# 34j/vr180-convert

Measured on NVIDIA B200. Metric: SBS equirect output Mpix/s, higher is better.
Workload: dtype f64 coordinates / u8 fixed-point (INTER_BITS=5) sampling

## Files before the change

### vr180-convert_b200/csrc/chain_fast.cuh

```cuda
#pragma once
#include "chain.cuh"

namespace vr180 {

static __device__ const double2 kAsinTab[92] = {
    {0x1.0000000000000p+0, 0x0.0p+0},
    {0x1.fffbfffbfff80p-1, 0x1.0000aaabdde0cp-7},
    {0x1.ffefffbffdfffp-1, 0x1.0002aabdde94cp-6},
    {0x1.ffdbfebbe9360p-1, 0x1.80090091d9024p-6},
    {0x1.ffbffbff7fec0p-1, 0x1.000aabde0b9c8p-5},
    {0x1.ff9bf63a1740bp-1, 0x1.4014d8ffaf8afp-5},
    {0x1.ff6febba4bfeap-1, 0x1.8024091fdb0a9p-5},
    {0x1.ff3bda6d9c950p-1, 0x1.c0393e65c2c93p-5},
    {0x1.feffbfdfebf1fp-1, 0x1.002abde953619p-4},
    {0x1.febb993aecf99p-1, 0x1.203ce2b380cd3p-4},
    {0x1.fe6f634576477p-1, 0x1.405390240e6fdp-4},
    {0x1.fe1b1a62bddadp-1, 0x1.606f49730ccc5p-4},
    {0x1.fdbeba917c3f5p-1, 0x1.809092913e52ep-4},
    {0x1.fd5a3f6af6b74p-1, 0x1.a0b7f03ba78acp-4},
    {0x1.fceda421efdb5p-1, 0x1.c0e5e80f7172dp-4},
    {0x1.fc78e3817e16ep-1, 0x1.e11b009e269b5p-4},
    {0x1.fbfbf7ebc755fp-1, 0x1.00abe0c129e1ep-3},
    {0x1.fb76db58a1299p-1, 0x1.10ce59ba4a8c4p-3},
    {0x1.fae987541497fp-1, 0x1.20f530308cc20p-3},
    {0x1.fa53f4fcc4b79p-1, 0x1.3120a9bed2f46p-3},
    {0x1.f9b61d0237250p-1, 0x1.41510cb011423p-3},
    {0x1.f90ff7a2fd4d2p-1, 0x1.5186a00ade974p-3},
    {0x1.f8617caabd6f6p-1, 0x1.61c1ab9d55d30p-3},
    {0x1.f7aaa3701a270p-1, 0x1.720278094cd3cp-3},
    {0x1.f6eb62d27730dp-1, 0x1.82494ed0e78fcp-3},
    {0x1.f623b1379a09bp-1, 0x1.92967a638db38p-3},
    {0x1.f553848924e81p-1, 0x1.a2ea462b4998ep-3},
    {0x1.f47ad231ea746p-1, 0x1.b344fe9a97c4dp-3},
    {0x1.f3998f1b1886cp-1, 0x1.c3a6f13aae84bp-3},
    {0x1.f2afafa9380f9p-1, 0x1.d4106cba45b08p-3},
    {0x1.f1bd27b9002c4p-1, 0x1.e481c0fce7134p-3},
    {0x1.f0c1ea9bfa45fp-1, 0x1.f4fb3f2ad079bp-3},
    {0x1.efbdeb14f4edap-1, 0x1.02be9ce0b87cdp-2},
    {0x1.eeb11b5442ff1p-1, 0x1.0b04025245cccp-2},
    {0x1.ed9b6cf3c4663p-1, 0x1.134dfa9805147p-2},
    {0x1.ec7cd0f2b5ae0p-1, 0x1.1b9cb12545e62p-2},
    {0x1.eb5537b1434dap-1, 0x1.23f0523c5dc2bp-2},
    {0x1.ea2490ebdd6b8p-1, 0x1.2c490af8bde81p-2},
    {0x1.e8eacbb648910p-1, 0x1.34a709597aab1p-2},
    {0x1.e7a7d6766784bp-1, 0x1.3d0a7c4c4bd9cp-2},
    {0x1.e65b9edeba38ep-1, 0x1.457393b90e2aap-2},
    {0x1.e50611e88d6b5p-1, 0x1.4de2808dce513p-2},
    {0x1.e3a71bcdd63dep-1, 0x1.565774cb66f02p-2},
    {0x1.e23ea802b4b1ap-1, 0x1.5ed2a392bb50fp-2},
    {0x1.e0cca12e97895p-1, 0x1.675441329986ep-2},
    {0x1.df50f124fba75p-1, 0x1.6fdc83364f719p-2},
    {0x1.ddcb80ddc085bp-1, 0x1.786ba074fef93p-2},
    {0x1.dc3c386d0ae09p-1, 0x1.8101d121bed2dp-2},
    {0x1.daa2fefaae1d8p-1, 0x1.899f4edc962d3p-2},
    {0x1.d8ffbab9145d4p-1, 0x1.924454c462cc4p-2},
    {0x1.d75250db9c792p-1, 0x1.9af11f89ba61cp-2},
    {0x1.d59aa58c6471cp-1, 0x1.a3a5ed82d9537p-2},
    {0x1.d3d89be176072p-1, 0x1.ac62fec0b2a92p-2},
    {0x1.d20c15d14a4e5p-1, 0x1.b5289525368abp-2},
    {0x1.d034f42698214p-1, 0x1.bdf6f47ae6904p-2},
    {0x1.ce5316736032ep-1, 0x1.c6ce628dd132cp-2},
    {0x1.cc665b0328622p-1, 0x1.cfaf27460fe9fp-2},
    {0x1.ca6e9ecc569b9p-1, 0x1.d8998cc3e6049p-2},
    {0x1.c86bbd609a260p-1, 0x1.e18ddf7da106bp-2},
    {0x1.c65d90dc509f4p-1, 0x1.ea8c6e5f5e67fp-2},
    {0x1.c443f1d4d22afp-1, 0x1.f3958aecddef4p-2},
    {0x1.c21eb7458e5ccp-1, 0x1.fca989658baafp-2},
    {0x1.bfedb67be13b3p-1, 0x1.02e46075785a1p-1},
    {0x1.bdb0c30185485p-1, 0x1.0779c5d4df4b8p-1},
    {0x1.bb67ae8584caap-1, 0x1.0c152382d7366p-1},
    {0x1.b91248c38986bp-1, 0x1.10b6a9e43942fp-1},
    {0x1.b6b05f6966b9bp-1, 0x1.155e8b2a00052p-1},
    {0x1.b441bdfab5580p-1, 0x1.1a0cfb6c3e9ebp-1},
    {0x1.b1c62db2564fep-1, 0x1.1ec230c714a96p-1},
    {0x1.af3d7561a9c43p-1, 0x1.237e6379cdfc7p-1},
    {0x1.aca7594d44cbdp-1, 0x1.2841ce0862975p-1},
    {0x1.aa039b06e926dp-1, 0x1.2d0cad5f90e20p-1},
    {0x1.a751f9447b724p-1, 0x1.31df40fbd31cdp-1},
    {0x1.a4922fb3ac8c2p-1, 0x1.36b9cb13786e1p-1},
    {0x1.a1c3f6ca01f29p-1, 0x1.3b9c90c43296dp-1},
    {0x1.9ee70390dec3dp-1, 0x1.4087da4473296p-1},
    {0x1.9bfb076d236ebp-1, 0x1.457bf318fe517p-1},
    {0x1.98ffafe1ece2fp-1, 0x1.4a792a4f26152p-1},
    {0x1.95f4a64decda8p-1, 0x1.4f7fd2bc2fb34p-1},
    {0x1.92d98fa2c355ep-1, 0x1.5490434275b92p-1},
    {0x1.8fae0c15ad38ap-1, 0x1.59aad71ced00fp-1},
    {0x1.8c71b6c8c49b4p-1, 0x1.5ecfee31c96e7p-1},
    {0x1.8924256bf4545p-1, 0x1.63ffed6d198f6p-1},
    {0x1.85c4e7d4a0bb1p-1, 0x1.693b3f244ee17p-1},
    {0x1.8253878ae2e09p-1, 0x1.6e825383cc40bp-1},
    {0x1.7ecf874b086dfp-1, 0x1.73d5a107bde74p-1},
    {0x1.7b386279d7bf3p-1, 0x1.7935a501afa78p-1},
    {0x1.778d8c89dc27cp-1, 0x1.7ea2e42c9027ap-1},
    {0x1.73ce704fb7b23p-1, 0x1.841deb5114bb4p-1},
    {0x1.6ffa6f4323c0dp-1, 0x1.89a74ffcc34a4p-1},
    {0x1.6c10e0a9e5d65p-1, 0x1.8f3fb14e496b4p-1},
    {0x1.681110a985d4dp-1, 0x1.94e7b8da3cf7ap-1},
};
constexpr double kPio2Hi = 0x1.921fb54442d18p+0, kPio2Lo = 0x1.1a62633145c07p-54;

__device__ __forceinline__ double theta_unit(double vz, double h) {
    const double az = fabs(vz);
    const bool swap = az > h;
    const double u = swap ? h : az, w = swap ? az : h;
    const int i = min(__double2int_rn(u * 128.0), 91);
    const double2 t = __ldg(kAsinTab + i);
    const double d = fma(u, t.x, -(w * ((double)i * 0.0078125)));
    const double d2 = d * d;
    double p = fma(d2, 15.0 / 336.0, 3.0 / 40.0);
    p = fma(d2, p, 1.0 / 6.0);
    const double al = t.y + fma(d, p * d2, d);
    const bool neg = vz < 0.0;
    const double k = swap ? (neg ? 2.0 : 0.0) : 1.0;
    double th = fma(k, kPio2Hi, swap == neg ? -al : al);
    th = fma(k, kPio2Lo, th);
    return az <= 1.0 ? th : CUDART_NAN;
}

constexpr int kStdTableDoubles = 7 * 32;
__device__ __forceinline__ void std_tables(const double* R, bool lat_is_y, bool is_row, double sv, double cv, double* x_side,
                                           double* y_side, int idx) {
    const bool is_x = lat_is_y == is_row;
    if (is_x) {
        const int o = lat_is_y ? 1 : 0;
        x_side[idx] = cv;
        x_side[32 + idx] = R[o] * sv;
        x_side[64 + idx] = R[3 + o] * sv;
        x_side[96 + idx] = R[6 + o] * sv;
    } else {
        const int o = lat_is_y ? 0 : 1;
        y_side[idx] = fma(R[o], sv, R[2] * cv);
        y_side[32 + idx] = fma(R[3 + o], sv, R[5] * cv);
        y_side[64 + idx] = fma(R[6 + o], sv, R[8] * cv);
    }
}

template <bool NORMALISED>
__device__ __forceinline__ void std_pixel(double vx, double vy, double vz, const double* poly, int n_poly, const double* den,
                                          double& ox, double& oy) {
    const double h2 = fma(vx, vx, vy * vy);
    double ux = 0.0, uy = 1.0, h = h2;
    if (h2 > 0.0) {
        const double inv = rsqrt(h2);
        ux = vx * inv;
        uy = vy * inv;
        h = h2 * inv;
    }
    double r = theta_unit(vz, h);
    if (r == 0.0) {
        ux = 1.0;
        uy = 0.0;
    }
    if (n_poly >= 0) {
        static_assert(VR180_MAX_OP_PARAMS == 12, "extend the chain below");
        double acc = 0.0;
#define VR180_HORNER(i) acc = fma(acc, r, poly[i]);
        switch (n_poly) {
            default: VR180_HORNER(11)
            case 11: VR180_HORNER(10)
            case 10: VR180_HORNER(9)
            case 9: VR180_HORNER(8)
            case 8: VR180_HORNER(7)
            case 7: VR180_HORNER(6)
            case 6: VR180_HORNER(5)
            case 5: VR180_HORNER(4)
            case 4: VR180_HORNER(3)
            case 3: VR180_HORNER(2)
            case 2: VR180_HORNER(1)
            case 1: VR180_HORNER(0)
            case 0: break;
        }
#undef VR180_HORNER
        r = acc;
    }
    r *= kTwoOverPi;
    if (NORMALISED) {
        ox = r * ux;
        oy = r * uy;
    } else {
        ox = fma(r * den[0], ux, den[2]);
        oy = fma(r * den[1], uy, den[3]);
    }
}

}
```

### vr180-convert_b200/csrc/stream.cu

```cuda
#include "tiled.cuh"

namespace vr180 {
namespace tiled {

constexpr int kSlots = 3;
constexpr int kSlowCap = 128;
constexpr int kStreamCtas = 3;

template <class M>
struct SLay {
    static constexpr int kSlotBytes = kStreamSlotBytes<M>;
    static_assert(kSlots == 3, "kStreamSlotBytes (tiled.cuh) is a third of the staging area");
    static constexpr int kOutTileBytes = M::kTileH * kTileW * 3;
    static constexpr int kOB = kOutBufs;
    static constexpr int kOutItemBytes = 2 * kOutTileBytes;
    static constexpr int kOffOut = kSlots * kSlotBytes;
    static constexpr int kOffBar = kOffOut + kOB * kOutItemBytes;
    static constexpr int kOffQ = (kOffBar + (kSlots + 2 * kOB) * 8 + 15) & ~15;
    static constexpr int kOffW = (kOffQ + kSlots * 16 + 15) & ~15;
    static constexpr int kWeightTab = M::kInterp == VR180_INTER_LINEAR ? 1024 * 8 : 0;
    static constexpr int kOffTab = kOffW + M::kWeightSmem;
    static constexpr int kOffSlow = kOffTab + kWeightTab;
    static constexpr int kSmemBytes = kOffSlow + kSlowCap * 8;
};

struct StreamParams {
    int tiles_x, n_tiles, n_units;
    int zero_border;
    const short* tab;
};

struct UnitGeom {
    int fast, bx0, ry0, pitch, rsel, rect_bytes, org;
    int eye_pitch;
};
template <class M>
__device__ __forceinline__ UnitGeom unit_geom(const int4& raw, int zero_border, int src_cols, int src_rows) {
    UnitGeom g;
    const TileHdr h = decode_header(raw);
    const TileRect rc = tile_rect<M>(h.mnx, h.mxx, h.mny, h.mxy);
    g.bx0 = rc.bx0;
    g.org = 3 * (h.mnx - M::kLo) - rc.bx0;
    g.ry0 = rc.ry0;
    g.pitch = kPitchMin + kPitchStep * ((h.flags >> 8) & 15);
    g.rsel = (h.flags >> 12) & 15;
    g.rect_bytes = (M::kRowsMin + g.rsel * kRowsStep) * g.pitch;
    g.eye_pitch = (g.rect_bytes + 127) & ~127;
    constexpr int kAll = kHdrPackable | kHdrStageable | kHdrFitsSlot;
    g.fast = (h.flags & kAll) == kAll;
    if (!zero_border)
        g.fast = g.fast && (int)h.mnx - M::kLo >= 0 && (int)h.mxx + M::kHi <= src_cols - 1 && (int)h.mny - M::kLo >= 0 &&
                 (int)h.mxy + M::kHi <= src_rows - 1;
    return g;
}

template <int N>
struct Entries {
    uint32_t e[N];
};
template <class M>
__device__ __forceinline__ void gather_tile(const RemapArgs& a, const StreamParams& sp, int grp, int tile, int nv, bool packed,
                                         int mnx, int mny, Entries<M::kPx> ev) {
    constexpr int kPx = M::kPx;
    const int tid = threadIdx.x, lane = tid & 31, sw = tid >> 5;
    const ViewArgs& mv = a.view[grp];
    const int ty = tile / sp.tiles_x, tx = tile - ty * sp.tiles_x;
    const int x0 = tx * kTileW, y0 = ty * M::kTileH;
#pragma unroll
    for (int k = 0; k < kPx; ++k) {
        const int i = x0 + lane, j = y0 + kPx * sw + k;
        if (i >= a.W || j >= a.H) continue;
        int2 q;
        if (packed) {
            q = unpack_entry<M>(mnx, mny, ev.e[k]);
        } else {
            q.x = M::quant(__ldg(mv.xmap + (long long)j * mv.map_pitch + i));
            q.y = M::quant(__ldg(mv.ymap + (long long)j * mv.map_pitch + i));
        }
        for (int f = 0; f < a.n_frames; ++f) gather_pixel<M>(a, f, i, j, grp, grp + nv, q.x, q.y, sp.tab);
    }
}

template <class M>
__global__ void __launch_bounds__(kThreads, kStreamCtas)
k_warp_stream(const __grid_constant__ RemapArgs a, const __grid_constant__ StreamParams sp,
              const __grid_constant__ TmaMaps tm) {
    constexpr int kPx = M::kPx;
    constexpr int kOB = SLay<M>::kOB, kOutTileBytes = SLay<M>::kOutTileBytes, kSlotBytes = SLay<M>::kSlotBytes;
    constexpr int kOutItemBytes = SLay<M>::kOutItemBytes;
    extern __shared__ __align__(1024) uint8_t smem[];
    const int tid = threadIdx.x, lane = tid & 31, warp = tid >> 5;
    const uint32_t s_stage = smem_u32(smem), s_full = s_stage + SLay<M>::kOffBar;
    const uint32_t s_ofull = s_full + kSlots * 8, s_oempty = s_ofull + kOB * 8, s_out = s_stage + SLay<M>::kOffOut;
    int4* const s_q = reinterpret_cast<int4*>(smem + SLay<M>::kOffQ);
    if (tid < kSlots + 2 * kOB) {
        const bool by_warps = tid >= kSlots && tid < kSlots + kOB;
        mbar_init(s_full + tid * 8, by_warps ? kSamplers / 32 : 1);
        asm volatile("fence.mbarrier_init.release.cluster;" ::: "memory");
    }
    if constexpr (SLay<M>::kWeightTab != 0) {
        uint2* const wt = reinterpret_cast<uint2*>(smem + SLay<M>::kOffTab);
        for (int i = tid; i < 1024; i += kThreads) {
            typename M::Pixel p;
            M::weights(p, i & 31, i >> 5, nullptr);
            wt[i] = make_uint2(p.W01, p.W23);
        }
    }
    __syncthreads();
    const int nv = a.share_map ? a.n_views : 1;
    const int src_cols = a.view[0].cols, src_rows = a.view[0].rows;
    const int stride = gridDim.x;

    if (warp == kSamplers / 32) {
        if (lane != 0) return;
        int n_load = 0, n_store = 0, l_slot = 0, s_slot = 0;
        auto store_next = [&]() {
            const int o = n_store & (kOB - 1);
            mbar_wait(s_ofull + o * 8, (uint32_t)(n_store / kOB) & 1u);
            const int4 q = s_q[s_slot];
            tma_store_3d(&tm.dst, q.x, q.y, q.z & 0xffff, s_out + o * kOutItemBytes);
            if (q.w >= 0) tma_store_3d(&tm.dst, q.w, q.y, q.z >> 16, s_out + o * kOutItemBytes + kOutTileBytes);
            bulk_commit();
            bulk_wait_read<0>();
            mbar_arrive(s_oempty + o * 8);
            ++n_store;
            if (++s_slot == kSlots) s_slot = 0;
        };
        int grp_n = 0, tile_n = blockIdx.x;
        while (tile_n >= sp.n_tiles) { tile_n -= sp.n_tiles; ++grp_n; }
        int4 hn = packed_header_raw(a.view[grp_n].packed, tile_n);
        for (int u = blockIdx.x; u < sp.n_units; u += stride) {
            const int4 hdr = hn;
            const int grp = grp_n, tile = tile_n;
            tile_n += stride;
            while (tile_n >= sp.n_tiles) { tile_n -= sp.n_tiles; ++grp_n; }
            if (u + stride < sp.n_units) hn = packed_header_raw(a.view[grp_n].packed, tile_n);
            const UnitGeom g = unit_geom<M>(hdr, sp.zero_border, src_cols, src_rows);
            if (!g.fast) continue;
            const int ty = tile / sp.tiles_x, tx = tile - ty * sp.tiles_x;
            const CUtensorMap* const map0 = &tm.src[grp][(g.pitch - kPitchMin) / kPitchStep][g.rsel];
            const int n_rects = a.n_frames * nv, per_item = 2 * g.eye_pitch <= kSlotBytes ? 2 : 1;
            const int x_l = (a.view[grp].dst_x_offset + tx * kTileW) * 3;
            const int x_r = nv == 2 ? (a.view[grp + 1].dst_x_offset + tx * kTileW) * 3 : x_l;
            for (int r = 0; r < n_rects; r += per_item) {
                if (n_load - n_store == kSlots) store_next();
                const uint32_t bar = s_full + l_slot * 8;
                const uint32_t dst = s_stage + l_slot * kSlotBytes;
                const bool two = per_item == 2 && r + 1 < n_rects;
                const int v0 = nv == 2 ? (r & 1) : 0, f0 = nv == 2 ? (r >> 1) : r;
                const int v1 = nv == 2 ? ((r + 1) & 1) : 0, f1 = nv == 2 ? ((r + 1) >> 1) : r + 1;
                s_q[l_slot] = make_int4(v0 ? x_r : x_l, ty * M::kTileH, f0 | (f1 << 16), two ? (v1 ? x_r : x_l) : -1);
                mbar_expect_tx(bar, (two ? 2u : 1u) * (uint32_t)g.rect_bytes);
                tma_load_3d(dst, map0 + v0 * (kWidths * kRowSizes), g.bx0, g.ry0, f0, bar);
                if (two) tma_load_3d(dst + g.eye_pitch, map0 + v1 * (kWidths * kRowSizes), g.bx0, g.ry0, f1, bar);
                ++n_load;
                if (++l_slot == kSlots) l_slot = 0;
            }
        }
        while (n_store < n_load) store_next();
        bulk_wait_read<0>();
        return;
    }

    const int sw = warp;
    const int sub = lane & 3;
    const uint32_t out_sel = sub == 0 ? 0x4210u : (sub == 1 ? 0x5421u : 0x6542u);
    uint32_t outp = s_out + (kPx * sw) * (kTileW * 3) + (3 * (lane >> 2) + sub) * 4;
    uint32_t flags = (sub != 3 ? 1u : 0u) | (lane == 0 ? 2u : 0u);
    asm volatile("" : "+r"(outp), "+r"(flags));

    int2* const s_slow = reinterpret_cast<int2*>(smem + SLay<M>::kOffSlow);
    int n = 0, st = 0;
    uint32_t ph = 0;
    int grp_n = 0, tile_n = blockIdx.x;
    while (tile_n >= sp.n_tiles) { tile_n -= sp.n_tiles; ++grp_n; }
    int u = blockIdx.x;
  for (;;) {
    int n_slow = 0;
    int4 hn = packed_header_raw(a.view[grp_n].packed, tile_n);
    uint32_t en[kPx];
    load_packed_entries<M>(a.view[grp_n].packed, sp.n_tiles, tile_n, tid, en);
    for (; u < sp.n_units && n_slow < kSlowCap; u += stride) {
        const int4 hdr = hn;
        uint32_t e[kPx];
#pragma unroll
        for (int k = 0; k < kPx; ++k) e[k] = en[k];
        const int grp = grp_n, tile = tile_n;
        tile_n += stride;
        while (tile_n >= sp.n_tiles) { tile_n -= sp.n_tiles; ++grp_n; }
        if (u + stride < sp.n_units) {
            hn = packed_header_raw(a.view[grp_n].packed, tile_n);
            load_packed_entries<M>(a.view[grp_n].packed, sp.n_tiles, tile_n, tid, en);
        }
        const UnitGeom g = unit_geom<M>(hdr, sp.zero_border, src_cols, src_rows);

        if (!g.fast) {
            if (tid == 0) s_slow[n_slow] = make_int2(grp, tile);
            ++n_slow;
            continue;
        }

        typename M::Pixel pc[kPx];
#pragma unroll
        for (int k = 0; k < kPx; ++k) {
            const int dx = (int)(e[k] & 255u), dy = (int)((e[k] >> 8) & 255u);
            M::set_offset(pc[k], dy * g.pitch + 3 * dx + g.org, true);
            if constexpr (SLay<M>::kWeightTab != 0) {
                asm("ld.shared.v2.u32 {%0, %1}, [%2];"
                    : "=r"(pc[k].W01), "=r"(pc[k].W23)
                    : "r"(s_stage + SLay<M>::kOffTab + ((e[k] >> 13) & (1023u << 3))));
            } else {
                M::weights(pc[k], (int)((e[k] >> 16) & 31u), (int)((e[k] >> 21) & 31u), sp.tab);
            }
        }
        if constexpr (M::kWeightSmem != 0) {
            uint8_t* slot = smem + SLay<M>::kOffW + tid * 16;
#pragma unroll
            for (int ky = 0; ky < 8; ++ky)
                *reinterpret_cast<uint4*>(slot + ky * (kSamplers * 16)) = __ldg(reinterpret_cast<const uint4*>(pc[0].w) + ky);
            pc[0].ws = smem_u32(slot);
        }

        const int n_rects = a.n_frames * nv, per_item = 2 * g.eye_pitch <= kSlotBytes ? 2 : 1;
        auto item_loop = [&](auto rects_tag, int n_items) {
            constexpr int EYES = decltype(rects_tag)::value;
#pragma unroll 1
            for (int it = 0; it < n_items; ++it) {
                mbar_wait(s_full + st * 8, ph);
                const uint32_t buf = s_stage + st * kSlotBytes;
                const int o = n & (kOB - 1);
                const uint32_t ob = outp + o * kOutItemBytes;
#pragma unroll
                for (int v = 0; v < EYES; ++v) {
                    uint32_t word[kPx];
#pragma unroll
                    for (int k = 0; k < kPx; ++k) {
                        const uint32_t r = M::sample(buf + v * g.eye_pitch, pc[k], (uint32_t)g.pitch);
                        word[k] = __byte_perm(r, __shfl_down_sync(0xffffffffu, r, 1), out_sel);
                    }
                    if (v == 0 && n >= kOB) mbar_wait(s_oempty + o * 8, (uint32_t)(n / kOB + 1) & 1u);
                    if (flags & 1u) {
#pragma unroll
                        for (int k = 0; k < kPx; ++k) sts32(ob + v * kOutTileBytes + k * (kTileW * 3), word[k]);
                    }
                }
                fence_proxy_async();
                __syncwarp();
                if (flags & 2u) mbar_arrive(s_ofull + o * 8);
                ++n;
                if (++st == kSlots) { st = 0; ph ^= 1u; }
            }
        };
        if (per_item == 2 && n_rects > 1) {
            item_loop(std::integral_constant<int, 2>{}, n_rects >> 1);
            if (n_rects & 1) item_loop(std::integral_constant<int, 1>{}, 1);
        } else {
            item_loop(std::integral_constant<int, 1>{}, n_rects);
        }
    }
    if (n_slow == 0 && u >= sp.n_units) break;
    asm volatile("bar.sync 1, %0;" ::"n"(kSamplers) : "memory");
    for (int i = 0; i < n_slow; ++i) {
        const int2 gt = s_slow[i];
        const int4 hdr = packed_header_raw(a.view[gt.x].packed, gt.y);
        Entries<kPx> ev;
        load_packed_entries<M>(a.view[gt.x].packed, sp.n_tiles, gt.y, tid, ev.e);
        const TileHdr h = decode_header(hdr);
        gather_tile<M>(a, sp, gt.x, gt.y, nv, (h.flags & kHdrPackable) != 0, h.mnx, h.mny, ev);
    }
    if (u >= sp.n_units) break;
    asm volatile("bar.sync 1, %0;" ::"n"(kSamplers) : "memory");
  }
}

template <class M>
static int launch_stream_mode(const RemapArgs& a, const short* tab, cudaStream_t st) {
    const int n_groups = a.share_map ? 1 : a.n_views;
    if (a.n_frames > 0x7fff) return VR180_ERR_UNSUPPORTED;
    const TmaMaps* tm = tma_maps_for(a, M::kInterp, M::kRowsMin, M::kTileH, 1);
    if (!tm) return VR180_ERR_UNSUPPORTED;
    int dev = 0;
    const int rc = max_dyn_smem_once<k_warp_stream<M>>(SLay<M>::kSmemBytes, dev);
    if (rc != VR180_OK) return rc;
    static std::atomic<int> sm_count[64];
    int sms = dev < 64 ? sm_count[dev].load(std::memory_order_acquire) : 0;
    if (!sms) {
        VR180_CUDA(cudaDeviceGetAttribute(&sms, cudaDevAttrMultiProcessorCount, dev));
        if (dev < 64) sm_count[dev].store(sms, std::memory_order_release);
    }
    StreamParams sp;
    memset(&sp, 0, sizeof(sp));
    sp.tiles_x = (a.W + kTileW - 1) / kTileW;
    const long long tiles = (long long)sp.tiles_x * ((a.H + M::kTileH - 1) / M::kTileH);
    if (tiles * n_groups > 0x7fffffffLL) return VR180_ERR_UNSUPPORTED;
    sp.n_tiles = (int)tiles;
    sp.n_units = (int)(tiles * n_groups);
    sp.zero_border = zero_border(a);
    sp.tab = tab;
    const int forced = g_debug_stream_grid.load(std::memory_order_relaxed);
    int grid = forced > 0 ? forced : sms * kStreamCtas;
    if (grid > sp.n_units) grid = sp.n_units;
    k_warp_stream<M><<<grid, kThreads, SLay<M>::kSmemBytes, st>>>(a, sp, *tm);
    g_launches.fetch_add(1, std::memory_order_relaxed);
    VR180_CUDA(cudaGetLastError());
    return VR180_OK;
}

}

int launch_remap_stream(const RemapArgs& a, int interp, const short* weight_tab, cudaStream_t st) {
    using namespace tiled;
    if (interp == VR180_INTER_NEAREST) return launch_stream_mode<Nearest>(a, nullptr, st);
    if (interp == VR180_INTER_LINEAR) return launch_stream_mode<LinearP>(a, nullptr, st);
    if (interp == VR180_INTER_CUBIC) return launch_stream_mode<Cubic>(a, weight_tab, st);
    if (interp == VR180_INTER_LANCZOS4) return launch_stream_mode<Lanczos4>(a, weight_tab, st);
    return VR180_ERR_UNSUPPORTED;
}

}
```

### vr180-convert_b200/csrc/tiled.cu

```cuda
#include "tiled.cuh"

namespace vr180 {
namespace tiled {

struct TileGeom {
    int rsel;
    int bx0, ry0;
    int x0, y0;
};

template <class M, int NV, bool DYN, int FR, bool SPLIT = false, bool VPAIR = false>
__device__ __forceinline__ void frame_loop(const RemapArgs& a, const TmaMaps& tm, int v_begin, int f0, int f1,
                                           const typename M::Pixel (&pc)[M::kPx], const TileGeom& tg, const int pitch,
                                           uint8_t* smem, int band, int cg, const DynRadius& dr,
                                           const double (&nx)[M::kPx], const double (&ny)[M::kPx], const short* tab) {
    static_assert(FR == 1 || !DYN, "a per-frame radius gives every frame its own rectangle");
    static_assert(M::kOutTiles / FR >= 2, "at least two out buffers of one item each");
    constexpr int kOutTileBytes = M::kTileH * kTileW * 3;
    constexpr int kOutItemBytes = FR * kOutTileBytes;
    constexpr int OB = M::kOutTiles / FR < kOutBufs ? M::kOutTiles / FR : kOutBufs;
    const int tid = threadIdx.x, lane = tid & 31, warp = tid >> 5;
    uint32_t s_stage = smem_u32(smem);
    asm volatile("" : "+r"(s_stage));
    const uint32_t s_full = s_stage + Lay<M>::kOffBar;
    const uint32_t s_ofull = s_full + 2 * kMaxStages * 8, s_oempty = s_ofull + kOutBufs * 8, s_out = s_stage + Lay<M>::kOffOut;

    int2* const s_org = reinterpret_cast<int2*>(smem + Lay<M>::kOffOrg);
    static_assert(!VPAIR || (SPLIT && FR == 2 && NV == 2 && !DYN), "an eye pair is two one-frame boxes of two views");
    const int n_items = VPAIR ? (f1 - f0) : ((f1 - f0 + FR - 1) / FR) * NV;
    const int rect_bytes = (M::kRowsMin + tg.rsel * kRowsStep) * pitch;
    const int stage_bytes = FR * rect_bytes;
    const int frame_pitch = SPLIT ? (rect_bytes + 127) & ~127 : rect_bytes;
    const int stage_stride = (FR * frame_pitch + 127) & ~127;
    static_assert(Lay<M>::kStageArea % 128 == 0 && Lay<M>::kStageArea / 128 <= 1024, "float quotient below");
    const int S = min(kMaxStages, (int)__fdividef((float)(Lay<M>::kStageArea / 128) + 0.5f, (float)(stage_stride >> 7)));

    if (warp == kSamplers / 32) {
        if (lane != 0) return;
        const CUtensorMap* const map0 = &tm.src[v_begin][(pitch - kPitchMin) / kPitchStep][tg.rsel];
        const int dst_x0 = (a.view[v_begin].dst_x_offset + tg.x0) * 3;
        const int dst_x1 = (a.view[v_begin + NV - 1].dst_x_offset + tg.x0) * 3;
        int p_item = 0, p_stage = 0;
        auto load = [&]() {
            const uint32_t bar = s_full + p_stage * 8;
            const int v = (NV == 2 && !VPAIR) ? (p_item & 1) : 0;
            const int f = VPAIR ? f0 + p_item : f0 + FR * ((NV == 2) ? (p_item >> 1) : p_item);
            int bx0 = tg.bx0, ry0 = tg.ry0;
            if (DYN) {
                const double rad = __ldg(dr.radius + f);
                if (rad == rad) {
                    int xlo, xhi, ylo, yhi;
                    dyn_range<M>(dr.ext[0], dr.ext[1], rad, dr.cx, xlo, xhi);
                    dyn_range<M>(dr.ext[2], dr.ext[3], rad, dr.cy, ylo, yhi);
                    const TileRect rc = tile_rect<M>(xlo, xhi, ylo, yhi);
                    bx0 = rc.bx0;
                    ry0 = rc.ry0;
                } else {
                    bx0 = ry0 = -(1 << 20);
                }
                s_org[p_stage] = make_int2(bx0, ry0);
            }
            mbar_expect_tx(bar, (uint32_t)stage_bytes);
            if (SPLIT) {
#pragma unroll
                for (int fr = 0; fr < FR; ++fr)
                    tma_load_3d(s_stage + p_stage * stage_stride + fr * frame_pitch,
                                map0 + (VPAIR ? fr : v) * (kWidths * kRowSizes), bx0, ry0, VPAIR ? f : f + fr, bar);
            } else {
                tma_load_3d(s_stage + p_stage * stage_stride, map0 + v * (kWidths * kRowSizes), bx0, ry0, f, bar);
            }
            ++p_item;
            if (++p_stage == S) p_stage = 0;
        };
        for (int n = 0; n < S && n < n_items; ++n) load();
        for (int n = 0; n < n_items; ++n) {
            const int o = n & (OB - 1);
            const int v = (NV == 2 && !VPAIR) ? (n & 1) : 0;
            const int f = VPAIR ? f0 + n : f0 + FR * ((NV == 2) ? (n >> 1) : n);
            mbar_wait(s_ofull + o * 8, (uint32_t)(n / OB) & 1u);
            if (n + S < n_items) load();
            if (SPLIT) {
#pragma unroll
                for (int fr = 0; fr < FR; ++fr)
                    tma_store_3d(&tm.dst, (VPAIR ? fr : v) ? dst_x1 : dst_x0, tg.y0, VPAIR ? f : f + fr,
                                 s_out + o * kOutItemBytes + fr * kOutTileBytes);
            } else {
                tma_store_3d(&tm.dst, v ? dst_x1 : dst_x0, tg.y0, f, s_out + o * kOutItemBytes);
            }
            bulk_commit();
            bulk_wait_read<0>();
            mbar_arrive(s_oempty + o * 8);
        }
        bulk_wait_read<0>();
        return;
    }

    const int sub = lane & 3;
    const uint32_t out_sel = sub == 0 ? 0x4210u : (sub == 1 ? 0x5421u : 0x6542u);
    const bool writer = sub != 3;
    constexpr int kOutStep = M::kRowPatch ? kTileW * 3 : 24;
    const int sw = band * (4 / M::kPx) + cg;
    uint32_t outp = s_out + (M::kRowPatch ? (M::kPx * sw) * (kTileW * 3) + (3 * (lane >> 2) + sub) * 4
                                          : (4 * band + (lane >> 3)) * (kTileW * 3) + M::kPx * cg * 24 +
                                                (3 * ((lane & 7) >> 2) + sub) * 4);
    uint32_t flags = (writer ? 1u : 0u) | (lane == 0 ? 2u : 0u);
    asm volatile("" : "+r"(outp), "+r"(flags));

    int st = 0;
    uint32_t ph = 0;
    typename M::Pixel cur[M::kPx];
    double cur_rad = CUDART_NAN;
    bool cur_have = false;
#pragma unroll
    for (int k = 0; k < M::kPx; ++k) cur[k] = pc[k];
    for (int n = 0; n < n_items; ++n) {
        mbar_wait(s_full + st * 8, ph);
        const uint32_t buf = s_stage + st * stage_stride;
        uint32_t res[FR][M::kPx];
        if (DYN) {
            const int f = f0 + ((NV == 2) ? (n >> 1) : n);
            const double rad = __ldg(dr.radius + f);
            if (!(rad == cur_rad)) {
                const int2 org = s_org[st];
                cur_have = rad == rad;
#pragma unroll
                for (int k = 0; k < M::kPx; ++k) {
                    const int qx = denorm_q<M>(nx[k], rad, dr.cx), qy = denorm_q<M>(ny[k], rad, dr.cy);
                    const int off = ((qy >> M::kShift) - M::kLo - org.y) * pitch + 3 * ((qx >> M::kShift) - M::kLo) - org.x;
                    M::set_offset(cur[k], off, cur_have);
                    M::weights(cur[k], qx & 31, qy & 31, tab);
                }
                cur_rad = rad;
            }
#pragma unroll
            for (int k = 0; k < M::kPx; ++k) {
                const uint32_t r = M::sample(buf, cur[k], (uint32_t)pitch);
                res[0][k] = cur_have ? r : 0u;
            }
        }
        uint32_t word[FR][M::kPx];
        if (!DYN && M::kInterp == VR180_INTER_LANCZOS4) {
#pragma unroll
            for (int k = 0; k < M::kPx; ++k) {
                uint32_t r[FR];
                sample_item<M, FR>(buf, (uint32_t)frame_pitch, pc[k], (uint32_t)pitch, r);
#pragma unroll
                for (int fr = 0; fr < FR; ++fr) res[fr][k] = r[fr];
            }
        }
#pragma unroll
        for (int fr = 0; fr < FR; ++fr) {
            if (!DYN && M::kInterp != VR180_INTER_LANCZOS4) {
#pragma unroll
                for (int k = 0; k < M::kPx; ++k) res[fr][k] = M::sample(buf + fr * frame_pitch, pc[k], (uint32_t)pitch);
            }
#pragma unroll
            for (int k = 0; k < M::kPx; ++k)
                word[fr][k] = __byte_perm(res[fr][k], __shfl_down_sync(0xffffffffu, res[fr][k], 1), out_sel);
        }
        const int o = n & (OB - 1);
        if (n >= OB) mbar_wait(s_oempty + o * 8, (uint32_t)(n / OB + 1) & 1u);
        if (flags & 1u) {
            const uint32_t ob = outp + o * kOutItemBytes;
#pragma unroll
            for (int fr = 0; fr < FR; ++fr)
#pragma unroll
                for (int k = 0; k < M::kPx; ++k) sts32(ob + fr * kOutTileBytes + k * kOutStep, word[fr][k]);
        }
        fence_proxy_async();
        __syncwarp();
        if (flags & 2u) mbar_arrive(s_ofull + o * 8);
        if (++st == S) { st = 0; ph ^= 1u; }
    }
}

template <class M, bool DYN, int FR>
__global__ void __launch_bounds__(kThreads, 4)
k_warp_tiled(const __grid_constant__ RemapArgs a, const __grid_constant__ vr180_chain_t chain0,
             const __grid_constant__ vr180_chain_t chain1, const __grid_constant__ TiledParams tp,
             const __grid_constant__ TmaMaps tm) {
    constexpr int kPx = M::kPx;
    constexpr int kChainUnroll = (FR == 1 && !DYN) ? kPx : 1;
    constexpr int kWarpsPerBand = 4 / kPx;
    extern __shared__ __align__(1024) uint8_t smem[];
    double* s_trig = reinterpret_cast<double*>(smem + Lay<M>::kOffTrig);
    int4* s_red = reinterpret_cast<int4*>(smem + Lay<M>::kOffRed);

    const int tid = threadIdx.x, lane = tid & 31, warp = tid >> 5;
    if (tid < 2 * kMaxStages + 2 * kOutBufs) {
        const uint32_t bars = smem_u32(smem + Lay<M>::kOffBar);
        const bool by_warps = (tid >= kMaxStages && tid < 2 * kMaxStages + kOutBufs);
        mbar_init(bars + tid * 8, by_warps ? kSamplers / 32 : 1);
        asm volatile("fence.mbarrier_init.release.cluster;" ::: "memory");
    }
    int* const s_cost = reinterpret_cast<int*>(smem + Lay<M>::kOffCost);
    if (tid < kPitchCands) s_cost[tid] = 0;
    const int tx = blockIdx.x, ty = blockIdx.y, tile = ty * tp.tiles_x + tx;
    const int x0 = tx * kTileW, y0 = ty * M::kTileH;
    const bool two_groups = !a.share_map && a.n_views == 2;
    const int g = two_groups ? (int)(blockIdx.z & 1u) : 0;
    const int chunk = two_groups ? (int)(blockIdx.z >> 1) : (int)blockIdx.z;
    const ViewArgs& mv = a.view[g];
    const int v_begin = g, v_end = a.share_map ? a.n_views : g + 1, nv = v_end - v_begin;
    const int f0 = chunk * a.frames_per_cta, f1 = min(a.n_frames, f0 + a.frames_per_cta);
    const bool sampler = warp < kSamplers / 32;
    const int sw = warp & (kSamplers / 32 - 1), band = sw / kWarpsPerBand, cg = sw % kWarpsPerBand;
    const int lx = M::kRowPatch ? lane : 8 * kPx * cg + (lane & 7), ly = M::kRowPatch ? kPx * sw : 4 * band + (lane >> 3);
    auto pcol = [&](int k) { return M::kRowPatch ? lx : lx + 8 * k; };
    auto prow = [&](int k) { return M::kRowPatch ? ly + k : ly; };
    const bool full_tile = (x0 + kTileW <= a.W) && (y0 + M::kTileH <= a.H);

    TileHdr hdr = {0, 0, 0, 0, 0};
    if (mv.map_kind != VR180_MAPSRC_ANALYTIC && mv.packed) hdr = decode_header(packed_header_raw(mv.packed, tile));
    const bool packed_tile = (hdr.flags & 1) != 0;

    int sx[kPx], sy[kPx];
    double nx[kPx], ny[kPx];
#pragma unroll
    for (int k = 0; k < kPx; ++k) {
        sx[k] = sy[k] = 0;
        nx[k] = ny[k] = 0.0;
    }
    constexpr bool dyn = DYN;
    if (mv.map_kind == VR180_MAPSRC_ANALYTIC) {
        const vr180_chain_t& ch = mv.chain_idx ? chain1 : chain0;
        const StdChain& sc = tp.std[mv.chain_idx ? 1 : 0];
        const bool fastc = sc.valid && sc.fast && !(tp.debug & 256);
        if (sc.valid || tp.sep_prefix) {
            if (tid < 64) {
                const bool is_row = tid >= 32;
                const int idx = tid & 31;
                const double* nm = ch.ops[0].p;
                const double c = (double)((is_row ? y0 : x0) + idx);
                const double n = mul_rn(__ddiv_rn(add_rn(c, -(is_row ? nm[1] : nm[0])), nm[2]), 2.0);
                double sv, cv;
                sincos(mul_rn(n, kHalfPi), &sv, &cv);
                if (fastc) {
                    std_tables(sc.R, sc.lat_is_y != 0, is_row, sv, cv, s_trig, s_trig + 128, idx);
                } else {
                    s_trig[(is_row ? 64 : 0) + idx] = sv;
                    s_trig[(is_row ? 96 : 32) + idx] = cv;
                }
            }
            __syncthreads();
            const bool lat_is_y = ch.ops[1].iparam != 0;
            auto seed = [&](int k, ChainState& s) {
                const double s_row = s_trig[64 + prow(k)], c_row = s_trig[96 + prow(k)];
                const double s_col = s_trig[pcol(k)], c_col = s_trig[32 + pcol(k)];
                s.mode = MODE_VEC3;
                s.x = s.y = s.r = s.ux = s.uy = 0.0;
                if (lat_is_y) {
                    s.vx = mul_rn(c_row, s_col);
                    s.vy = s_row;
                    s.vz = mul_rn(c_row, c_col);
                } else {
                    s.vx = s_col;
                    s.vy = mul_rn(c_col, s_row);
                    s.vz = mul_rn(c_col, c_row);
                }
            };
            if (!sampler) {
            } else if (fastc) {
                auto std_eval = [&](const StdChain& c) {
                    const bool x_fixed = M::kRowPatch ? !c.lat_is_y : (c.lat_is_y != 0);
                    const int fi = M::kRowPatch ? lx : ly;
                    const double* const ft = s_trig + (x_fixed ? 0 : 128) + fi;
                    const double f0 = ft[0], f1 = ft[32], f2 = ft[64], f3 = x_fixed ? ft[96] : 0.0;
#pragma unroll(kChainUnroll)
                    for (int k = 0; k < kPx; ++k) {
                        const int vi = M::kRowPatch ? prow(k) : pcol(k);
                        double vx, vy, vz;
                        if (x_fixed) {
                            vx = fma(f0, s_trig[128 + vi], f1); vy = fma(f0, s_trig[160 + vi], f2); vz = fma(f0, s_trig[192 + vi], f3);
                        } else {
                            const double sc_ = s_trig[vi];
                            vx = fma(sc_, f0, s_trig[32 + vi]); vy = fma(sc_, f1, s_trig[64 + vi]); vz = fma(sc_, f2, s_trig[96 + vi]);
                        }
                        double ox, oy;
                        int qx = 0, qy = 0;
                        if (dyn) {
                            std_pixel<true>(vx, vy, vz, c.poly, c.n_poly, c.den, ox, oy);
                        } else {
                            std_pixel<false>(vx, vy, vz, c.poly, c.n_poly, c.den, ox, oy);
                            qx = M::quant(__double2float_rn(ox));
                            qy = M::quant(__double2float_rn(oy));
                        }
#pragma unroll
                        for (int kk = 0; kk < kPx; ++kk)
                            if (kk == k) { sx[kk] = qx; sy[kk] = qy; nx[kk] = ox; ny[kk] = oy; }
                    }
                };
                if (mv.chain_idx) std_eval(tp.std[1]);
                else std_eval(tp.std[0]);
            } else {
#pragma unroll 1
                for (int k = 0; k < kPx; ++k) {
                    ChainState s;
                    seed(k, s);
                    run_ops(ch, 2, ch.n_ops - (dyn ? 1 : 0), s);
                    to_xy(s);
                    const int qx = M::quant(__double2float_rn(s.x)), qy = M::quant(__double2float_rn(s.y));
#pragma unroll
                    for (int kk = 0; kk < kPx; ++kk)
                        if (kk == k) { sx[kk] = qx; sy[kk] = qy; nx[kk] = s.x; ny[kk] = s.y; }
                }
            }
        } else if (sampler) {
#pragma unroll 1
            for (int k = 0; k < kPx; ++k) {
                double xs, ys;
                if (dyn) eval_chain_normalised(ch, x0 + pcol(k), y0 + prow(k), xs, ys);
                else eval_chain(ch, x0 + pcol(k), y0 + prow(k), xs, ys);
                const int qx = M::quant(__double2float_rn(xs)), qy = M::quant(__double2float_rn(ys));
#pragma unroll
                for (int kk = 0; kk < kPx; ++kk)
                    if (kk == k) { sx[kk] = qx; sy[kk] = qy; nx[kk] = xs; ny[kk] = ys; }
            }
        }
    } else if (sampler) {
        bool unpacked = false;
        {
            if (packed_tile) {
                uint32_t e[kPx];
                load_packed_entries<M>(mv.packed, tp.n_tiles, tile, tid, e);
#pragma unroll
                for (int k = 0; k < kPx; ++k) {
                    const int2 q = unpack_entry<M>(hdr.mnx, hdr.mny, e[k]);
                    sx[k] = q.x;
                    sy[k] = q.y;
                }
                unpacked = true;
            }
        }
#pragma unroll
        for (int k = 0; k < kPx; ++k) {
            if (unpacked) break;
            const int i = x0 + pcol(k), j = y0 + prow(k);
            sx[k] = sy[k] = (int)0x80000000;
            if (i < a.W && j < a.H) {
                if (mv.map_kind == VR180_MAPSRC_FLOAT2) {
                    sx[k] = M::quant(__ldg(mv.xmap + (long long)j * mv.map_pitch + i));
                    sy[k] = M::quant(__ldg(mv.ymap + (long long)j * mv.map_pitch + i));
                } else {
                    const int2 q = __ldg(mv.fixed + (long long)j * mv.map_pitch + i);
                    sx[k] = q.x;
                    sy[k] = q.y;
                }
            }
        }
    }

    bool dynr = dyn;
    if (dyn) {
        const vr180_chain_t& ch = mv.chain_idx ? chain1 : chain0;
        const double r0 = __ldg(mv.radius_dev + f0);
        int same = r0 == r0;
        for (int f = f0 + 1 + lane; f < f1; f += 32) same &= __ldg(mv.radius_dev + f) == r0;
        if (__all_sync(0xffffffffu, same)) {
            dynr = false;
            const double cx = ch.ops[ch.n_ops - 1].p[2], cy = ch.ops[ch.n_ops - 1].p[3];
#pragma unroll
            for (int k = 0; k < kPx; ++k) {
                sx[k] = denorm_q<M>(nx[k], r0, cx);
                sy[k] = denorm_q<M>(ny[k], r0, cy);
            }
        }
    }

    if (!packed_tile) block_box_store<M>(sx, sy, s_red, warp, lane == 0 && sampler);
    DynRadius dr;
    dr.radius = nullptr;
    dr.cx = dr.cy = 0.0;
    dr.ext[0] = dr.ext[1] = dr.ext[2] = dr.ext[3] = 0.0;
    int nan_px = 0;
    if (dynr) {
        double* s_ext = reinterpret_cast<double*>(smem + Lay<M>::kOffExt);
        double e0 = CUDART_INF, e1 = -CUDART_INF, e2 = CUDART_INF, e3 = -CUDART_INF;
        if (sampler) {
#pragma unroll
            for (int k = 0; k < kPx; ++k) {
                nan_px |= (nx[k] != nx[k]) | (ny[k] != ny[k]);
                e0 = fmin(e0, nx[k]);
                e1 = fmax(e1, nx[k]);
                e2 = fmin(e2, ny[k]);
                e3 = fmax(e3, ny[k]);
            }
        }
#pragma unroll
        for (int d = 16; d > 0; d >>= 1) {
            e0 = fmin(e0, __shfl_xor_sync(0xffffffffu, e0, d));
            e1 = fmax(e1, __shfl_xor_sync(0xffffffffu, e1, d));
            e2 = fmin(e2, __shfl_xor_sync(0xffffffffu, e2, d));
            e3 = fmax(e3, __shfl_xor_sync(0xffffffffu, e3, d));
        }
        if (lane == 0 && sampler) {
            s_ext[warp * 4 + 0] = e0;
            s_ext[warp * 4 + 1] = e1;
            s_ext[warp * 4 + 2] = e2;
            s_ext[warp * 4 + 3] = e3;
        }
    }
    nan_px = __syncthreads_or(nan_px);
    static_assert(Lay<M>::kOffRed % 16 == 0, "s_red is read as int4");
    const int4 box = packed_tile ? make_int4(hdr.mnx, hdr.mxx, hdr.mny, hdr.mxy) : block_box_load(s_red, lane);
    const int mnx = box.x, mxx = box.y, mny = box.z, mxy = box.w;
    const TileRect rc = tile_rect<M>(mnx, mxx, mny, mxy);
    const bool vpair = !DYN && FR == 1 && nv == 2;
    const int fr_item = dynr ? 1 : (vpair ? 2 : FR);
    auto stage_fits = [&](int box_rows, int pitch_bytes) {
        const int rect = box_rows * pitch_bytes;
        return ((fr_item * ((DYN || vpair) ? (rect + 127) & ~127 : rect) + 127) & ~127) <= Lay<M>::kStageArea;
    };
    const int src_cols = a.view[v_begin].cols, src_rows = a.view[v_begin].rows;
    auto inside_src = [&](int x_lo, int x_hi, int y_lo, int y_hi) {
        return x_lo - M::kLo >= 0 && x_hi + M::kHi <= src_cols - 1 && y_lo - M::kLo >= 0 && y_hi + M::kHi <= src_rows - 1;
    };
    bool fast = full_tile && rc.wbytes <= kPitchMax && rc.rsel < kRowSizes && mnx > -32768 && mny > -32768 &&
                mxx < 32767 && mxy < 32767 && stage_fits(rc.box_rows, max(rc.wbytes, kPitchMin)) &&
                (tp.zero_border || inside_src(mnx, mxx, mny, mxy));
    int dyn_wbytes = 0, dyn_nrows = 0;
    if (dynr) {
        const double* s_ext = reinterpret_cast<const double*>(smem + Lay<M>::kOffExt);
        dr.ext[0] = dr.ext[2] = CUDART_INF;
        dr.ext[1] = dr.ext[3] = -CUDART_INF;
#pragma unroll
        for (int w = 0; w < kSamplers / 32; ++w) {
            dr.ext[0] = fmin(dr.ext[0], s_ext[w * 4 + 0]);
            dr.ext[1] = fmax(dr.ext[1], s_ext[w * 4 + 1]);
            dr.ext[2] = fmin(dr.ext[2], s_ext[w * 4 + 2]);
            dr.ext[3] = fmax(dr.ext[3], s_ext[w * 4 + 3]);
        }
        const vr180_chain_t& ch = mv.chain_idx ? chain1 : chain0;
        dr.radius = mv.radius_dev;
        dr.cx = ch.ops[ch.n_ops - 1].p[2];
        dr.cy = ch.ops[ch.n_ops - 1].p[3];
        int ok = 1;
        for (int f = f0 + lane; f < f1; f += 32) {
            const double rad = __ldg(dr.radius + f);
            if (rad == rad) {
                int lo, hi, ylo, yhi;
                dyn_range<M>(dr.ext[0], dr.ext[1], rad, dr.cx, lo, hi);
                ok &= (lo > -32768) & (hi < 32767);
                dyn_range<M>(dr.ext[2], dr.ext[3], rad, dr.cy, ylo, yhi);
                ok &= (ylo > -32768) & (yhi < 32767);
                const TileRect rf = tile_rect<M>(lo, hi, ylo, yhi);
                dyn_wbytes = max(dyn_wbytes, rf.wbytes);
                dyn_nrows = max(dyn_nrows, rf.nrows);
                if (!tp.zero_border) ok &= inside_src(lo, hi, ylo, yhi) ? 1 : 0;
            } else if (!tp.zero_border) {
                ok = 0;
            }
        }
        dyn_wbytes = __reduce_max_sync(0xffffffffu, dyn_wbytes);
        dyn_nrows = __reduce_max_sync(0xffffffffu, dyn_nrows);
        ok = __all_sync(0xffffffffu, ok);
        fast = full_tile && ok && !nan_px && dyn_wbytes <= kPitchMax && box_rsel<M>(dyn_nrows) < kRowSizes &&
               stage_fits(M::kRowsMin + box_rsel<M>(dyn_nrows) * kRowsStep, max(dyn_wbytes, kPitchMin));
    }

    if (!fast) {
        if (sampler) {
#pragma unroll
            for (int k = 0; k < kPx; ++k) {
                const int i = x0 + pcol(k), j = y0 + prow(k);
                if (i < a.W && j < a.H) {
                    for (int f = f0; f < f1; ++f) {
                        int qx = sx[k], qy = sy[k];
                        if (dynr) {
                            const double rad = __ldg(dr.radius + f);
                            qx = denorm_q<M>(nx[k], rad, dr.cx);
                            qy = denorm_q<M>(ny[k], rad, dr.cy);
                        }
                        gather_pixel<M>(a, f, i, j, v_begin, v_end, qx, qy, tp.tab);
                    }
                }
            }
        }
        return;
    }

    int pitch = max(dynr ? dyn_wbytes : rc.wbytes, kPitchMin);
    if (!dynr && (f1 - f0) * nv >= 8) {
        if (sampler) pitch_costs<M>(sx[0], sy[0], rc, pitch, lane, s_cost);
        __syncthreads();
        pitch = pick_pitch(s_cost, pitch, rc.box_rows, [&](int pe) { return stage_fits(rc.box_rows, pe); });
    }

    typename M::Pixel pc[kPx];
#pragma unroll
    for (int k = 0; k < kPx; ++k) {
        const int ix = sx[k] >> M::kShift, iy = sy[k] >> M::kShift;
        const int off = (iy - M::kLo - rc.ry0) * pitch + 3 * (ix - M::kLo) - rc.bx0;
        M::set_offset(pc[k], off, true);
        if (sampler && !dynr) M::weights(pc[k], sx[k] & 31, sy[k] & 31, tp.tab);
    }
    if constexpr (M::kWeightSmem != 0) {
        if (!dynr && sampler) {
            uint8_t* slot = smem + Lay<M>::kOffW + tid * 16;
#pragma unroll
            for (int ky = 0; ky < 8; ++ky)
                *reinterpret_cast<uint4*>(slot + ky * (kSamplers * 16)) = __ldg(reinterpret_cast<const uint4*>(pc[0].w) + ky);
            pc[0].ws = smem_u32(slot);
        }
    }
    TileGeom tg;
    tg.rsel = dynr ? box_rsel<M>(dyn_nrows) : rc.rsel;
    tg.bx0 = rc.bx0;
    tg.ry0 = rc.ry0;
    tg.x0 = x0;
    tg.y0 = y0;
    if (DYN && dynr) {
        if (nv == 2) frame_loop<M, 2, DYN, 1>(a, tm, v_begin, f0, f1, pc, tg, pitch, smem, band, cg, dr, nx, ny, tp.tab);
        else         frame_loop<M, 1, DYN, 1>(a, tm, v_begin, f0, f1, pc, tg, pitch, smem, band, cg, dr, nx, ny, tp.tab);
    } else {
        if constexpr (!DYN && FR == 1) {
            if (nv == 2) frame_loop<M, 2, false, 2, true, true>(a, tm, v_begin, f0, f1, pc, tg, pitch, smem, band, cg, dr, nx, ny, tp.tab);
            else         frame_loop<M, 1, false, 1, false>(a, tm, v_begin, f0, f1, pc, tg, pitch, smem, band, cg, dr, nx, ny, tp.tab);
        } else {
            if (nv == 2) frame_loop<M, 2, false, FR, DYN>(a, tm, v_begin, f0, f1, pc, tg, pitch, smem, band, cg, dr, nx, ny, tp.tab);
            else         frame_loop<M, 1, false, FR, DYN>(a, tm, v_begin, f0, f1, pc, tg, pitch, smem, band, cg, dr, nx, ny, tp.tab);
        }
    }
}

template <class M>
__global__ void __launch_bounds__(kSamplers) k_pack_tiles(const float* __restrict__ xmap, const float* __restrict__ ymap,
                                                         long long map_pitch, int W, int H, int tiles_x, int n_tiles,
                                                         void* __restrict__ packed) {
    constexpr int kPx = M::kPx;
    __shared__ int4 s_red[kSamplers / 32];
    __shared__ int s_cost[kPitchCands];
    const int tid = threadIdx.x, lane = tid & 31, sw = tid >> 5;
    const int tx = blockIdx.x % tiles_x, ty = blockIdx.x / tiles_x;
    const int x0 = tx * kTileW, y0 = ty * M::kTileH;
    const bool full_tile = (x0 + kTileW <= W) && (y0 + M::kTileH <= H);
    if (tid < kPitchCands) s_cost[tid] = 0;
    int sx[kPx], sy[kPx];
#pragma unroll
    for (int k = 0; k < kPx; ++k) {
        const int i = x0 + lane, j = y0 + kPx * sw + k;
        sx[k] = sy[k] = (int)0x80000000;
        if (i < W && j < H) {
            sx[k] = M::quant(__ldg(xmap + (long long)j * map_pitch + i));
            sy[k] = M::quant(__ldg(ymap + (long long)j * map_pitch + i));
        }
    }
    block_box_store<M>(sx, sy, s_red, sw, lane == 0);
    __syncthreads();
    const int4 box = block_box_load(s_red, lane);
    const int mnx = box.x, mxx = box.y, mny = box.z, mxy = box.w;
    const bool ok = full_tile && mnx > -32768 && mny > -32768 && mxx < 32767 && mxy < 32767 && mxx - mnx <= 255 &&
                    mxy - mny <= 255;
    const TileRect rc = tile_rect<M>(mnx, mxx, mny, mxy);
    const bool stageable = ok && rc.wbytes <= kPitchMax && rc.rsel < kRowSizes;
    const int pitch0 = max(rc.wbytes, kPitchMin);
    if (stageable) pitch_costs<M>(sx[0], sy[0], rc, pitch0, lane, s_cost);
    __syncthreads();
    const int pitch = !stageable ? kPitchMin : pick_pitch(s_cost, pitch0, rc.box_rows, [&](int pe) {
        return pe == pitch0 || rc.box_rows * pe <= kStreamSlotBytes<M>;
    });
    const int widx = (pitch - kPitchMin) / kPitchStep;
    if (tid == 0) {
        int4 h;
        h.x = (mnx & 0xffff) | (mxx << 16);
        h.y = (mny & 0xffff) | (mxy << 16);
        h.z = (ok ? kHdrPackable : 0) | (stageable ? kHdrStageable : 0) |
              (stageable && rc.box_rows * pitch <= kStreamSlotBytes<M> ? kHdrFitsSlot : 0) | (widx << 8) | (rc.rsel << 12);
        h.w = 0;
        reinterpret_cast<int4*>(packed)[blockIdx.x] = h;
    }
    uint32_t* ent = reinterpret_cast<uint32_t*>(static_cast<uint8_t*>(packed) + packed_entries_offset(n_tiles)) +
                    ((size_t)blockIdx.x * kSamplers + tid) * kPx;
#pragma unroll
    for (int k = 0; k < kPx; ++k) {
        const int ix = sat16(sx[k] >> M::kShift), iy = sat16(sy[k] >> M::kShift);
        const uint32_t fx = M::kShift ? (uint32_t)(sx[k] & 31) : 0u, fy = M::kShift ? (uint32_t)(sy[k] & 31) : 0u;
        ent[k] = ok ? ((uint32_t)(ix - mnx) | ((uint32_t)(iy - mny) << 8) | (fx << 16) | (fy << 21)) : 0u;
    }
}

}

static int tile_height_of(int interp) {
    return interp == VR180_INTER_LINEAR || interp == VR180_INTER_NEAREST ? tiled::LinearP::kTileH
           : interp == VR180_INTER_CUBIC                                  ? tiled::Cubic::kTileH
           : interp == VR180_INTER_LANCZOS4                               ? tiled::Lanczos4::kTileH
                                                                          : 0;
}

size_t packed_lut_bytes(int out_w, int out_h, int interp) {
    const int th = tile_height_of(interp);
    if (!th) return 0;
    const long long n_tiles = (long long)((out_w + tiled::kTileW - 1) / tiled::kTileW) * ((out_h + th - 1) / th);
    return tiled::packed_entries_offset(n_tiles) + (size_t)n_tiles * tiled::kTileW * th * 4;
}

int launch_pack_lut_tiles(const float* xmap, const float* ymap, int64_t map_pitch, int W, int H, int interp, void* packed,
                          cudaStream_t st) {
    using namespace tiled;
    const int th = tile_height_of(interp);
    if (!th) return VR180_ERR_UNSUPPORTED;
    const int tiles_x = (W + kTileW - 1) / kTileW, tiles_y = (H + th - 1) / th;
    const long long n_tiles = (long long)tiles_x * tiles_y;
    if (n_tiles > 0x7fffffffLL) return VR180_ERR_UNSUPPORTED;
    const dim3 grid((unsigned)n_tiles);
    if (interp == VR180_INTER_NEAREST)
        k_pack_tiles<Nearest><<<grid, kSamplers, 0, st>>>(xmap, ymap, (long long)map_pitch, W, H, tiles_x, (int)n_tiles, packed);
    else if (interp == VR180_INTER_LINEAR)
        k_pack_tiles<LinearP><<<grid, kSamplers, 0, st>>>(xmap, ymap, (long long)map_pitch, W, H, tiles_x, (int)n_tiles, packed);
    else if (interp == VR180_INTER_CUBIC)
        k_pack_tiles<Cubic><<<grid, kSamplers, 0, st>>>(xmap, ymap, (long long)map_pitch, W, H, tiles_x, (int)n_tiles, packed);
    else
        k_pack_tiles<Lanczos4><<<grid, kSamplers, 0, st>>>(xmap, ymap, (long long)map_pitch, W, H, tiles_x, (int)n_tiles, packed);
    g_launches.fetch_add(1, std::memory_order_relaxed);
    VR180_CUDA(cudaGetLastError());
    return VR180_OK;
}

static void match_std_chain(const vr180_chain_t& c, tiled::StdChain& out) {
    memset(&out, 0, sizeof(out));
    out.n_poly = -1;
    if (c.n_ops < 4 || c.ops[0].code != VR180_OP_NORMALIZE || c.ops[1].code != VR180_OP_EQUIRECT_ENC) return;
    memcpy(out.norm, c.ops[0].p, sizeof(out.norm));
    out.lat_is_y = c.ops[1].iparam != 0;
    int k = 2;
    if (c.ops[k].code == VR180_OP_ROT3) {
        out.has_rot = 1;
        memcpy(out.R, c.ops[k].p, sizeof(out.R));
        ++k;
    }
    if (k < c.n_ops && c.ops[k].code == VR180_OP_POLY) {
        out.n_poly = c.ops[k].iparam;
        memcpy(out.poly, c.ops[k].p, sizeof(out.poly));
        ++k;
    }
    if (k + 2 != c.n_ops || c.ops[k].code != VR180_OP_FISHEYE_DEC || c.ops[k].iparam != VR180_MAP_EQUIDISTANT ||
        c.ops[k + 1].code != VR180_OP_DENORMALIZE)
        return;
    memcpy(out.den, c.ops[k + 1].p, sizeof(out.den));
    out.valid = 1;
    if (!out.has_rot) {
        out.R[0] = out.R[4] = out.R[8] = 1.0;
        out.fast = 1;
    } else {
        double err = 0.0;
        for (int i = 0; i < 3; ++i)
            for (int j = 0; j < 3; ++j) {
                double d = i == j ? -1.0 : 0.0;
                for (int m = 0; m < 3; ++m) d += out.R[3 * m + i] * out.R[3 * m + j];
                err = std::fmax(err, std::fabs(d));
            }
        out.fast = err < 1e-12 ? 1 : 0;
    }
}

using EncodeTiledFn = CUresult (*)(CUtensorMap*, CUtensorMapDataType, cuuint32_t, void*, const cuuint64_t*,
                                   const cuuint64_t*, const cuuint32_t*, const cuuint32_t*, CUtensorMapInterleave,
                                   CUtensorMapSwizzle, CUtensorMapL2promotion, CUtensorMapFloatOOBfill);

static EncodeTiledFn encode_tiled_fn() {
    static EncodeTiledFn fn = [] {
        void* p = nullptr;
        cudaDriverEntryPointQueryResult q = cudaDriverEntryPointSymbolNotFound;
        if (cudaGetDriverEntryPoint("cuTensorMapEncodeTiled", &p, cudaEnableDefault, &q) != cudaSuccess ||
            q != cudaDriverEntryPointSuccess)
            p = nullptr;
        cudaGetLastError();
        return reinterpret_cast<EncodeTiledFn>(p);
    }();
    return fn;
}

static bool encode_u8_3d(CUtensorMap* out, const void* base, long long row_bytes, long long rows, long long frames,
                         long long pitch, long long frame_stride, int box_w, int box_h, int box_d) {
    EncodeTiledFn fn = encode_tiled_fn();
    if (!fn) return false;
    if (frames <= 1 || frame_stride < pitch * rows) frame_stride = ((pitch * rows + 15) / 16) * 16;
    const cuuint64_t dims[3] = {(cuuint64_t)row_bytes, (cuuint64_t)rows, (cuuint64_t)(frames < 1 ? 1 : frames)};
    const cuuint64_t strides[2] = {(cuuint64_t)pitch, (cuuint64_t)frame_stride};
    const cuuint32_t box[3] = {(cuuint32_t)box_w, (cuuint32_t)box_h, (cuuint32_t)box_d};
    const cuuint32_t estr[3] = {1u, 1u, 1u};
    return fn(out, CU_TENSOR_MAP_DATA_TYPE_UINT8, 3, const_cast<void*>(base), dims, strides, box, estr,
              CU_TENSOR_MAP_INTERLEAVE_NONE, CU_TENSOR_MAP_SWIZZLE_NONE, CU_TENSOR_MAP_L2_PROMOTION_L2_128B,
              CU_TENSOR_MAP_FLOAT_OOB_FILL_NONE) == CUDA_SUCCESS;
}

int tiled_debug_flags() {
    static const int env_debug = [] { const char* e = getenv("VR180_TILED_DEBUG"); return e ? atoi(e) : 0; }();
    const int set_debug = g_debug_tiled_flags.load(std::memory_order_relaxed);
    return set_debug >= 0 ? set_debug : env_debug;
}

constexpr int kMaxFramesPerCta = 64;
static int frames_per_cta(long long tiles, int n_frames, int views_per_cta = 1) {
    const int forced = g_debug_frames_per_cta.load(std::memory_order_relaxed);
    if (forced > 0) return forced < n_frames ? forced : n_frames;
    const int cap_set = g_debug_max_frames_per_cta.load(std::memory_order_relaxed);
    const int cap = cap_set > 0 ? cap_set : kMaxFramesPerCta / views_per_cta;
    int fpc = n_frames;
    if (fpc > cap) fpc = (n_frames + (n_frames + cap - 1) / cap - 1) / ((n_frames + cap - 1) / cap);
    while (fpc > 1 && tiles * ((n_frames + fpc - 1) / fpc) < 148LL * 4 * 2) fpc = (fpc + 1) / 2;
    return fpc;
}

const tiled::TmaMaps* tma_maps_for(const RemapArgs& a0, int interp, int rows_min, int tile_h, int fr) {
    using namespace tiled;
    struct Key {
        const void* src[2];
        long long pitch[2], fs[2];
        int rows, cols, n_views, n_frames, H, mode, fr, pad;
        const void* dst;
        long long dst_pitch, dst_fs;
    };
    Key key;
    memset(&key, 0, sizeof(key));
    for (int v = 0; v < a0.n_views; ++v) {
        key.src[v] = a0.view[v].src;
        key.pitch[v] = a0.view[v].pitch;
        key.fs[v] = a0.view[v].frame_stride;
    }
    key.rows = a0.view[0].rows;
    key.cols = a0.view[0].cols;
    key.n_views = a0.n_views;
    key.n_frames = a0.n_frames;
    key.H = a0.H;
    key.mode = interp;
    key.fr = fr;
    key.dst = a0.dst;
    key.dst_pitch = a0.dst_pitch;
    key.dst_fs = a0.dst_frame_stride;
    struct Entry {
        Key key;
        TmaMaps tm;
        uint64_t stamp;
    };
    constexpr size_t kCacheEntries = 8;
    static thread_local std::vector<Entry> cache;
    static thread_local uint64_t clock_ = 0;
    Entry* hit = nullptr;
    for (Entry& e : cache)
        if (memcmp(&key, &e.key, sizeof(key)) == 0) hit = &e;
    if (!hit) {
        if (cache.size() < kCacheEntries) {
            cache.emplace_back();
            hit = &cache.back();
        } else {
            hit = &cache[0];
            for (Entry& e : cache)
                if (e.stamp < hit->stamp) hit = &e;
        }
        memset(&hit->key, 0xff, sizeof(hit->key));
        TmaMaps& t = hit->tm;
        memset(&t, 0, sizeof(t));
        for (int v = 0; v < a0.n_views; ++v) {
            const ViewArgs& vw = a0.view[v];
            for (int w = 0; w < kWidths; ++w)
                for (int r = 0; r < kRowSizes; ++r)
                    if (!encode_u8_3d(&t.src[v][w][r], vw.src, (long long)vw.cols * 3, vw.rows, a0.n_frames, vw.pitch,
                                      vw.frame_stride, kPitchMin + w * kPitchStep, rows_min + r * kRowsStep, fr))
                        return nullptr;
        }
        if (a0.n_views == 1) memcpy(&t.src[1], &t.src[0], sizeof(t.src[0]));
        if (!encode_u8_3d(&t.dst, a0.dst, a0.dst_pitch, a0.H, a0.n_frames, a0.dst_pitch, a0.dst_frame_stride, kTileW * 3,
                          tile_h, fr))
            return nullptr;
        hit->key = key;
    }
    hit->stamp = ++clock_;
    return &hit->tm;
}

template <class M, bool DYN, int FR>
static int launch_mode(const RemapArgs& a0, const vr180_chain_t& c0, const vr180_chain_t& c1, const short* tab,
                       cudaStream_t st) {
    using namespace tiled;
    const int n_groups = a0.share_map ? 1 : a0.n_views;
    const TmaMaps* tmp = tma_maps_for(a0, M::kInterp, M::kRowsMin, M::kTileH, DYN ? 1 : FR);
    if (!tmp) return VR180_ERR_UNSUPPORTED;
    const TmaMaps& tm = *tmp;

    int dev = 0;
    const int rc = max_dyn_smem_once<k_warp_tiled<M, DYN, FR>>(Lay<M>::kSmemBytes, dev);
    if (rc != VR180_OK) return rc;

    RemapArgs a = a0;
    TiledParams tp;
    memset(&tp, 0, sizeof(tp));
    const int tiles_x = (a.W + kTileW - 1) / kTileW, tiles_y = (a.H + M::kTileH - 1) / M::kTileH;
    tp.tiles_x = tiles_x;
    tp.n_tiles = tiles_x * tiles_y;
    tp.tab = tab;
    tp.zero_border = zero_border(a);
    tp.debug = tiled_debug_flags();
    const long long tiles = (long long)tiles_x * tiles_y * n_groups;
    int fpc = frames_per_cta(tiles, a.n_frames, a.share_map ? a.n_views : 1);
    fpc = (fpc + FR - 1) / FR * FR;
    a.frames_per_cta = fpc;
    const int chunks = (a.n_frames + fpc - 1) / fpc;
    if (n_groups > 2 || chunks * n_groups > 65535 || tiles_y > 65535 || tiles_x * (long long)tiles_y > 0x7fffffffLL)
        return VR180_ERR_UNSUPPORTED;
    auto is_sep = [](const vr180_chain_t& c) {
        return c.n_ops >= 2 && c.ops[0].code == VR180_OP_NORMALIZE && c.ops[1].code == VR180_OP_EQUIRECT_ENC;
    };
    tp.sep_prefix = 1;
    for (int g = 0; g < n_groups; ++g) {
        if (a.view[g].map_kind != VR180_MAPSRC_ANALYTIC) continue;
        const vr180_chain_t& c = a.view[g].chain_idx ? c1 : c0;
        if (!is_sep(c)) tp.sep_prefix = 0;
        match_std_chain(c, tp.std[a.view[g].chain_idx ? 1 : 0]);
    }
    dim3 grid((unsigned)tiles_x, (unsigned)tiles_y, (unsigned)(n_groups * chunks));
    k_warp_tiled<M, DYN, FR><<<grid, kThreads, Lay<M>::kSmemBytes, st>>>(a, c0, c1, tp, tm);
    g_launches.fetch_add(1, std::memory_order_relaxed);
    VR180_CUDA(cudaGetLastError());
    return VR180_OK;
}

template <class M>
static int launch_tiled(const RemapArgs& a0, const vr180_chain_t& c0, const vr180_chain_t& c1, const short* tab, bool dyn,
                        int fpc, cudaStream_t st) {
    if constexpr (M::kInterp == VR180_INTER_CUBIC) {
        if (fpc >= 8) return dyn ? launch_mode<M, true, 4>(a0, c0, c1, tab, st) : launch_mode<M, false, 4>(a0, c0, c1, tab, st);
    }
    if (fpc >= 2) return dyn ? launch_mode<M, true, 2>(a0, c0, c1, tab, st) : launch_mode<M, false, 2>(a0, c0, c1, tab, st);
    return dyn ? launch_mode<M, true, 1>(a0, c0, c1, tab, st) : launch_mode<M, false, 1>(a0, c0, c1, tab, st);
}

int launch_remap_tiled(const RemapArgs& a0, int channels, int interp, const vr180_chain_t& c0, const vr180_chain_t& c1,
                       const short* weight_tab, cudaStream_t st) {
    if (channels != 3 || a0.depth != VR180_DEPTH_8U) return VR180_ERR_UNSUPPORTED;
    if (interp != VR180_INTER_NEAREST && interp != VR180_INTER_LINEAR && interp != VR180_INTER_CUBIC &&
        interp != VR180_INTER_LANCZOS4)
        return VR180_ERR_UNSUPPORTED;
    if (interp == VR180_INTER_NEAREST)
        for (int v = 0; v < a0.n_views; ++v)
            if (a0.view[v].map_kind == VR180_MAPSRC_FIXED) return VR180_ERR_UNSUPPORTED;
    const int n_groups = a0.share_map ? 1 : a0.n_views;
    for (int v = 0; v < a0.n_views; ++v) {
        const ViewArgs& vw = a0.view[v];
        if (((uintptr_t)vw.src & 15) || (vw.pitch & 15) || (vw.frame_stride & 15) || vw.pitch < (long long)vw.cols * 3)
            return VR180_ERR_UNSUPPORTED;
        if (a0.n_frames > 1 && vw.frame_stride < vw.pitch * vw.rows) return VR180_ERR_UNSUPPORTED;
        if (vw.rows != a0.view[0].rows || vw.cols != a0.view[0].cols) return VR180_ERR_UNSUPPORTED;
        if ((vw.dst_x_offset * 3) & 15) return VR180_ERR_UNSUPPORTED;
    }
    if (((uintptr_t)a0.dst & 15) || (a0.dst_pitch & 15) || (a0.dst_frame_stride & 15)) return VR180_ERR_UNSUPPORTED;
    if (a0.n_frames > 1 && a0.dst_frame_stride < a0.dst_pitch * a0.H) return VR180_ERR_UNSUPPORTED;
    int n_dyn = 0;
    for (int g = 0; g < n_groups; ++g)
        n_dyn += (a0.view[g].map_kind == VR180_MAPSRC_ANALYTIC && a0.view[g].radius_dev) ? 1 : 0;
    if (n_dyn != 0 && n_dyn != n_groups) return VR180_ERR_UNSUPPORTED;
    const bool dyn = n_dyn != 0;
    const int kStreamMaxItems = a0.share_map ? 20 : 16;
    {
        bool all_packed = !dyn;
        for (int g = 0; g < n_groups; ++g) all_packed = all_packed && a0.view[g].packed != nullptr;
        const int dbg = tiled_debug_flags();
        const int items = a0.n_frames * (a0.share_map ? a0.n_views : 1);
        const bool tab_ok = (interp != VR180_INTER_CUBIC && interp != VR180_INTER_LANCZOS4) || weight_tab != nullptr;
        if (all_packed && tab_ok && !(dbg & 4) && ((dbg & 2) || items <= kStreamMaxItems) &&
            g_debug_frames_per_cta.load(std::memory_order_relaxed) <= 0) {
            const int rc = launch_remap_stream(a0, interp, weight_tab, st);
            if (rc != VR180_ERR_UNSUPPORTED) return rc;
        }
    }
    const int tile_h = tile_height_of(interp);
    const long long tiles = (long long)((a0.W + tiled::kTileW - 1) / tiled::kTileW) * ((a0.H + tile_h - 1) / tile_h) * n_groups;
    const int fpc = frames_per_cta(tiles, a0.n_frames, a0.share_map ? a0.n_views : 1);
    if (interp == VR180_INTER_NEAREST) return launch_tiled<tiled::Nearest>(a0, c0, c1, nullptr, dyn, fpc, st);
    if (interp == VR180_INTER_LINEAR) return launch_tiled<tiled::LinearP>(a0, c0, c1, nullptr, dyn, fpc, st);
    if (!weight_tab) return VR180_ERR_UNSUPPORTED;
    if (interp == VR180_INTER_LANCZOS4) return launch_tiled<tiled::Lanczos4>(a0, c0, c1, weight_tab, dyn, fpc, st);
    return launch_tiled<tiled::Cubic>(a0, c0, c1, weight_tab, dyn, fpc, st);
}

}
```

### vr180-convert_b200/csrc/tiled.cuh

```cuda
#pragma once
#include <cuda.h>

#include <cmath>
#include <cstdlib>
#include <mutex>
#include <type_traits>
#include <vector>

#include "chain_fast.cuh"
#include "common.cuh"
#include "sampler.cuh"

namespace vr180 {
namespace tiled {

constexpr int kTileW = 32;
constexpr int kSamplers = 256;
constexpr int kThreads = kSamplers + 32;
constexpr int kMaxStages = 8;
constexpr int kRowsStep = 4, kRowSizes = 9;
constexpr int kPitchMin = 96, kPitchMax = 256, kPitchStep = 16;
constexpr int kWidths = (kPitchMax - kPitchMin) / kPitchStep + 1;
constexpr int kPitchCands = 4;
constexpr int kStageAreaDefault = 40960;
constexpr int kOutBufs = 4;
template <class M>
struct Lay {
    static constexpr int kStageArea = M::kStageArea;
    static constexpr int kOutArea = M::kOutTiles * M::kTileH * kTileW * 3;
    static constexpr int kOffOut = kStageArea;
    static constexpr int kOffTrig = kOffOut + kOutArea;
    static constexpr int kOffRed = kOffTrig + 7 * 32 * 8;
    static constexpr int kOffBar = kOffRed + 8 * 4 * 4;
    static constexpr int kOffOrg = kOffBar + (2 * kMaxStages + 2 * kOutBufs) * 8;
    static constexpr int kOffExt = kOffOrg + kMaxStages * 8;
    static constexpr int kOffCost = kOffExt + 8 * 4 * 8;
    static constexpr int kOffW = (kOffCost + 16 + 15) & ~15;
    static constexpr int kSmemBytes = kOffW + M::kWeightSmem;
};

template <class M>
constexpr int kStreamSlotBytes = (M::kStageArea / 3) & ~127;

struct StdChain {
    int valid, lat_is_y, has_rot, n_poly;
    int fast, pad_;
    double norm[3];
    double R[9];
    double poly[VR180_MAX_OP_PARAMS];
    double den[4];
};

struct TiledParams {
    int tiles_x;
    int n_tiles;
    int sep_prefix;
    int debug;
    int zero_border;
    const short* tab;
    StdChain std[2];
};

struct alignas(64) TmaMaps {
    CUtensorMap src[2][kWidths][kRowSizes];
    CUtensorMap dst;
};

struct PackedHdr {
    short mnx, mxx, mny, mxy;
    int flags;
    int pad;
};
constexpr int kHdrPackable = 1;
constexpr int kHdrStageable = 2;
constexpr int kHdrFitsSlot = 4;
static_assert(sizeof(PackedHdr) == 16, "PackedHdr is one 128-bit load");
__host__ __device__ inline size_t packed_entries_offset(long long n_tiles) { return ((size_t)n_tiles * 16 + 255) & ~(size_t)255; }
__device__ __forceinline__ int4 packed_header_raw(const void* packed, int tile) {
    return __ldg(reinterpret_cast<const int4*>(packed) + tile);
}
struct TileHdr {
    int mnx, mxx, mny, mxy, flags;
};
__device__ __forceinline__ TileHdr decode_header(const int4& v) {
    return {(short)(v.x & 0xffff), v.x >> 16, (short)(v.y & 0xffff), v.y >> 16, v.z};
}
template <class M>
__device__ __forceinline__ void load_packed_entries(const void* packed, int n_tiles, int tile, int tid, uint32_t (&e)[M::kPx]) {
    const uint32_t* ent = reinterpret_cast<const uint32_t*>(static_cast<const uint8_t*>(packed) + packed_entries_offset(n_tiles)) +
                          ((size_t)tile * kSamplers + tid) * M::kPx;
    if constexpr (M::kPx == 4) {
        const uint4 v = __ldg(reinterpret_cast<const uint4*>(ent));
        e[0] = v.x; e[1] = v.y; e[2] = v.z; e[3] = v.w;
    } else if constexpr (M::kPx == 2) {
        const uint2 v = __ldg(reinterpret_cast<const uint2*>(ent));
        e[0] = v.x; e[1] = v.y;
    } else {
        e[0] = __ldg(ent);
    }
}
template <class M>
__device__ __forceinline__ int2 unpack_entry(int hdr_mnx, int hdr_mny, uint32_t e) {
    return make_int2(((hdr_mnx + (int)(e & 255u)) << M::kShift) | (int)((e >> 16) & 31u),
                     ((hdr_mny + (int)((e >> 8) & 255u)) << M::kShift) | (int)((e >> 21) & 31u));
}

__device__ __forceinline__ uint32_t smem_u32(const void* p) { return (uint32_t)__cvta_generic_to_shared(p); }

__device__ __forceinline__ void mbar_init(uint32_t bar, uint32_t count) {
    asm volatile("mbarrier.init.shared::cta.b64 [%0], %1;" ::"r"(bar), "r"(count) : "memory");
}
__device__ __forceinline__ void mbar_expect_tx(uint32_t bar, uint32_t bytes) {
    asm volatile("mbarrier.arrive.expect_tx.shared::cta.b64 _, [%0], %1;" ::"r"(bar), "r"(bytes) : "memory");
}
__device__ __forceinline__ void mbar_arrive(uint32_t bar) {
    asm volatile("mbarrier.arrive.shared::cta.b64 _, [%0];" ::"r"(bar) : "memory");
}
constexpr uint32_t kSuspendNs = 4000;
__device__ __forceinline__ void mbar_wait(uint32_t bar, uint32_t parity) {
    asm volatile(
        "{\n\t.reg .pred p;\n\t"
        "WAIT_%=:\n\t"
        "mbarrier.try_wait.parity.shared::cta.b64 p, [%0], %1, %2;\n\t"
        "@p bra DONE_%=;\n\t"
        "bra WAIT_%=;\n\t"
        "DONE_%=:\n\t}" ::"r"(bar), "r"(parity), "r"(kSuspendNs)
        : "memory");
}
__device__ __forceinline__ void fence_proxy_async() { asm volatile("fence.proxy.async.shared::cta;" ::: "memory"); }
__device__ __forceinline__ void tma_load_3d(uint32_t dst, const CUtensorMap* map, int x, int y, int z, uint32_t bar) {
    asm volatile(
        "cp.async.bulk.tensor.3d.shared::cluster.global.tile.mbarrier::complete_tx::bytes [%0], [%1, {%2, %3, %4}], [%5];" ::
            "r"(dst), "l"(map), "r"(x), "r"(y), "r"(z), "r"(bar)
        : "memory");
}
__device__ __forceinline__ void tma_store_3d(const CUtensorMap* map, int x, int y, int z, uint32_t src) {
    asm volatile("cp.async.bulk.tensor.3d.global.shared::cta.tile.bulk_group [%0, {%1, %2, %3}], [%4];" ::"l"(map), "r"(x),
                 "r"(y), "r"(z), "r"(src)
                 : "memory");
}
__device__ __forceinline__ void bulk_commit() { asm volatile("cp.async.bulk.commit_group;" ::: "memory"); }
template <int N>
__device__ __forceinline__ void bulk_wait_read() {
    asm volatile("cp.async.bulk.wait_group.read %0;" ::"n"(N) : "memory");
}

__device__ __forceinline__ void sts32(uint32_t addr, uint32_t v) {
    asm volatile("st.shared.u32 [%0], %1;" ::"r"(addr), "r"(v) : "memory");
}

__device__ __forceinline__ uint32_t pack_sat_u8x3(int c0, int c1, int c2) {
    uint32_t t, d;
    asm("cvt.pack.sat.u8.s32.b32 %0, %1, %2, %3;" : "=r"(t) : "r"(0), "r"(c2), "r"(0));
    asm("cvt.pack.sat.u8.s32.b32 %0, %1, %2, %3;" : "=r"(d) : "r"(c1), "r"(c0), "r"(t));
    return d;
}

__device__ __forceinline__ uint32_t dp2a_lo_su(uint32_t w, uint32_t px, uint32_t acc) {
    uint32_t d;
    asm("dp2a.lo.s32.u32 %0, %1, %2, %3;" : "=r"(d) : "r"(w), "r"(px), "r"(acc));
    return d;
}
__device__ __forceinline__ uint32_t dp2a_hi_su(uint32_t w, uint32_t px, uint32_t acc) {
    uint32_t d;
    asm("dp2a.hi.s32.u32 %0, %1, %2, %3;" : "=r"(d) : "r"(w), "r"(px), "r"(acc));
    return d;
}

struct LinearP {
    static constexpr int kPx = 4, kTileH = 32, kLo = 0, kHi = 1, kRowsMin = 32, kInterp = VR180_INTER_LINEAR;
    static constexpr int kShift = kInterBits;
    __device__ static __forceinline__ int quant(float m) { return quantise(m); }
    static constexpr int kStageArea = kStageAreaDefault, kWeightSmem = 0, kOutTiles = 4;
    static constexpr bool kRowPatch = true;
    struct Pixel {
        uint32_t osel;
        uint32_t selT;
        uint32_t W01, W23;
    };
    __device__ static __forceinline__ void set_offset(Pixel& p, int off, bool valid) {
        const uint32_t s = (uint32_t)off & 3u;
        p.osel = ((valid ? ((uint32_t)off & ~3u) : 0u) << 16) | (0x30u + 0x11u * s);
        p.selT = (0x5241u + 0x1111u * s) & 0x7fffu;
    }
    __device__ static __forceinline__ void weights(Pixel& p, int ax, int ay, const short*) {
        const int w00 = (32 - ax) * (32 - ay), w01 = ax * (32 - ay), w10 = (32 - ax) * ay, w11 = ax * ay;
        p.W01 = (uint32_t)min(64 * w00, 65535) | ((uint32_t)(64 * w01) << 16);
        p.W23 = (uint32_t)(64 * w10) | ((uint32_t)(64 * w11) << 16);
    }
    __device__ static __forceinline__ uint32_t sample(uint32_t sbuf, const Pixel& p, uint32_t pitch) {
        const uint32_t row0 = sbuf + (p.osel >> 16);
        uint32_t q0, t0, t1;
        asm volatile(
            "{\n\t.reg .pred p;\n\t.reg .b32 a0, a1, b0, b1, u0, u1;\n\t"
            "setp.eq.u32 p, %6, 0x574;\n\t"
            "ld.shared.u32 a0, [%3];\n\t"
            "ld.shared.u32 a1, [%3+4];\n\t"
            "ld.shared.u32 b0, [%4];\n\t"
            "ld.shared.u32 b1, [%4+4];\n\t"
            "prmt.b32 u0, a0, a1, %5;\n\t"
            "prmt.b32 u1, b0, b1, %5;\n\t"
            "@p ld.shared.u32 a0, [%3+8];\n\t"
            "@p ld.shared.u32 b0, [%4+8];\n\t"
            "prmt.b32 %0, u0, u1, 0x5410;\n\t"
            "prmt.b32 %1, a0, a1, %6;\n\t"
            "prmt.b32 %2, b0, b1, %6;\n\t}"
            : "=&r"(q0), "=&r"(t0), "=&r"(t1)
            : "r"(row0), "r"(row0 + pitch), "r"(p.osel), "r"(p.selT));
        const uint32_t s0 = __dp2a_hi(p.W23, q0, __dp2a_lo(p.W01, q0, 32768u));
        const uint32_t s1 = __dp2a_lo(p.W23, t1, __dp2a_lo(p.W01, t0, 32768u));
        const uint32_t s2 = __dp2a_hi(p.W23, t1, __dp2a_hi(p.W01, t0, 32768u));
        return __byte_perm(__byte_perm(s0, s1, 0x0062), s2, 0x7610);
    }
};

struct Nearest {
    static constexpr int kPx = 4, kTileH = 32, kLo = 0, kHi = 0, kRowsMin = 32, kInterp = VR180_INTER_NEAREST;
    static constexpr int kShift = 0;
    __device__ static __forceinline__ int quant(float m) { return cv_round(m); }
    static constexpr int kStageArea = kStageAreaDefault, kWeightSmem = 0, kOutTiles = 4;
    static constexpr bool kRowPatch = true;
    struct Pixel {
        int boff;
        int sh;
    };
    __device__ static __forceinline__ void set_offset(Pixel& p, int off, bool valid) {
        p.boff = valid ? (off & ~3) : 0;
        p.sh = (off & 3) * 8;
    }
    __device__ static __forceinline__ void weights(Pixel&, int, int, const short*) {}
    __device__ static __forceinline__ uint32_t sample(uint32_t sbuf, const Pixel& p, uint32_t) {
        uint32_t a0, a1;
        asm volatile("ld.shared.u32 %0, [%2];\n\tld.shared.u32 %1, [%2+4];" : "=r"(a0), "=r"(a1) : "r"(sbuf + (uint32_t)p.boff));
        return __funnelshift_r(a0, a1, p.sh);
    }
};

struct Cubic {
    static constexpr int kPx = 2, kTileH = 16, kLo = 1, kHi = 2, kRowsMin = 16, kInterp = VR180_INTER_CUBIC;
    static constexpr int kShift = kInterBits;
    __device__ static __forceinline__ int quant(float m) { return quantise(m); }
    static constexpr int kStageArea = kStageAreaDefault, kWeightSmem = 0, kOutTiles = 8;
    static constexpr bool kRowPatch = true;
    struct Pixel {
        int boff;
        int sh;
        uint32_t w[8];
    };
    __device__ static __forceinline__ void set_offset(Pixel& p, int off, bool valid) {
        p.boff = valid ? (off & ~3) : 0;
        p.sh = (off & 3) * 8;
    }
    __device__ static __forceinline__ void weights(Pixel& p, int ax, int ay, const short* tab) {
        const uint4* t = reinterpret_cast<const uint4*>(tab + ((ay << 5) | ax) * 16);
        const uint4 lo = __ldg(t), hi = __ldg(t + 1);
        p.w[0] = lo.x; p.w[1] = lo.y; p.w[2] = lo.z; p.w[3] = lo.w;
        p.w[4] = hi.x; p.w[5] = hi.y; p.w[6] = hi.z; p.w[7] = hi.w;
    }
    __device__ static __forceinline__ uint32_t sample(uint32_t sbuf, const Pixel& p, uint32_t pitch) {
        const uint32_t* r = reinterpret_cast<const uint32_t*>(
            static_cast<const uint8_t*>(__cvta_shared_to_generic(sbuf)) + p.boff);
        const int sh = p.sh;
        uint32_t acc0 = 16384u, acc1 = 16384u, acc2 = 16384u;
#pragma unroll
        for (int ky = 0; ky < 4; ++ky, r += pitch / 4) {
            const uint32_t a0 = r[0], a1 = r[1], a2 = r[2], a3 = r[3];
            const uint32_t A0 = __funnelshift_r(a0, a1, sh), A1 = __funnelshift_r(a1, a2, sh),
                           A2 = __funnelshift_r(a2, a3, sh);
            const uint32_t q0 = __byte_perm(__byte_perm(A0, A1, 0x0630), A2, 0x5210);
            const uint32_t q1 = __byte_perm(__byte_perm(A0, A1, 0x0741), A2, 0x6210);
            const uint32_t q2 = __byte_perm(__byte_perm(A0, A1, 0x0052), A2, 0x7410);
            const uint32_t w01 = p.w[2 * ky], w23 = p.w[2 * ky + 1];
            acc0 = dp2a_hi_su(w23, q0, dp2a_lo_su(w01, q0, acc0));
            acc1 = dp2a_hi_su(w23, q1, dp2a_lo_su(w01, q1, acc1));
            acc2 = dp2a_hi_su(w23, q2, dp2a_lo_su(w01, q2, acc2));
        }
        return pack_sat_u8x3((int)acc0 >> 15, (int)acc1 >> 15, (int)acc2 >> 15);
    }
};

struct Lanczos4 {
    static constexpr int kPx = 1, kTileH = 8, kLo = 3, kHi = 4, kRowsMin = 16, kInterp = VR180_INTER_LANCZOS4;
    static constexpr bool kRowPatch = true;
    static constexpr int kShift = kInterBits;
    __device__ static __forceinline__ int quant(float m) { return quantise(m); }
    static constexpr int kStageArea = 16384, kWeightSmem = kSamplers * 128;
    static constexpr int kOutTiles = 4;
    struct Pixel {
        int boff;
        int sh;
        const short* w;
        uint32_t ws;
    };
    __device__ static __forceinline__ void set_offset(Pixel& p, int off, bool valid) {
        p.boff = valid ? (off & ~3) : 0;
        p.sh = (off & 3) * 8;
    }
    __device__ static __forceinline__ void weights(Pixel& p, int ax, int ay, const short* tab) {
        p.w = tab + (((ay << 5) | ax) << 6);
        p.ws = 0;
    }
    template <int NF>
    __device__ static __forceinline__ void sample_frames(uint32_t sbuf, uint32_t frame_bytes, const Pixel& p, uint32_t pitch,
                                                         uint32_t (&out)[NF]) {
        const uint8_t* base = static_cast<const uint8_t*>(__cvta_shared_to_generic(sbuf)) + p.boff;
        const int sh = p.sh;
        uint32_t acc[NF][3];
#pragma unroll
        for (int f = 0; f < NF; ++f) acc[f][0] = acc[f][1] = acc[f][2] = 16384u;
#pragma unroll
        for (int ky = 0; ky < 8; ++ky) {
            uint4 wv;
            if (p.ws) {
                asm volatile("ld.shared.v4.u32 {%0, %1, %2, %3}, [%4];"
                             : "=r"(wv.x), "=r"(wv.y), "=r"(wv.z), "=r"(wv.w)
                             : "r"(p.ws + ky * (kSamplers * 16)));
            } else {
                wv = __ldg(reinterpret_cast<const uint4*>(p.w + ky * 8));
            }
            const uint32_t wp[4] = {wv.x, wv.y, wv.z, wv.w};
#pragma unroll
            for (int f = 0; f < NF; ++f) {
                const uint32_t* r = reinterpret_cast<const uint32_t*>(base + f * frame_bytes + ky * pitch);
                uint32_t x[7], A[6];
#pragma unroll
                for (int i = 0; i < 7; ++i) x[i] = r[i];
#pragma unroll
                for (int i = 0; i < 6; ++i) A[i] = __funnelshift_r(x[i], x[i + 1], sh);
#pragma unroll
                for (int g = 0; g < 2; ++g) {
                    const uint32_t A0 = A[3 * g], A1 = A[3 * g + 1], A2 = A[3 * g + 2];
                    const uint32_t q0 = __byte_perm(__byte_perm(A0, A1, 0x0630), A2, 0x5210);
                    const uint32_t q1 = __byte_perm(__byte_perm(A0, A1, 0x0741), A2, 0x6210);
                    const uint32_t q2 = __byte_perm(__byte_perm(A0, A1, 0x0052), A2, 0x7410);
                    acc[f][0] = dp2a_hi_su(wp[2 * g + 1], q0, dp2a_lo_su(wp[2 * g], q0, acc[f][0]));
                    acc[f][1] = dp2a_hi_su(wp[2 * g + 1], q1, dp2a_lo_su(wp[2 * g], q1, acc[f][1]));
                    acc[f][2] = dp2a_hi_su(wp[2 * g + 1], q2, dp2a_lo_su(wp[2 * g], q2, acc[f][2]));
                }
            }
        }
#pragma unroll
        for (int f = 0; f < NF; ++f) {
            out[f] = pack_sat_u8x3((int)acc[f][0] >> 15, (int)acc[f][1] >> 15, (int)acc[f][2] >> 15);
        }
    }
    __device__ static __forceinline__ uint32_t sample(uint32_t sbuf, const Pixel& p, uint32_t pitch) {
        uint32_t out[1];
        sample_frames<1>(sbuf, 0u, p, pitch, out);
        return out[0];
    }
};

struct DynRadius {
    const double* radius;
    double cx, cy;
    double ext[4];
};
template <class M>
__device__ __forceinline__ int denorm_q(double n, double rad, double c) {
    return M::quant(__double2float_rn(add_rn(mul_rn(n, rad), c)));
}
template <class M>
__device__ __forceinline__ void dyn_range(double nmin, double nmax, double rad, double c, int& lo, int& hi) {
    const int a = sat16(denorm_q<M>(nmin, rad, c) >> M::kShift), b = sat16(denorm_q<M>(nmax, rad, c) >> M::kShift);
    lo = min(a, b);
    hi = max(a, b);
}

template <class M>
__device__ __forceinline__ void block_box_store(const int (&sx)[M::kPx], const int (&sy)[M::kPx], int4* s_red, int warp,
                                                bool store) {
    int mnx = INT_MAX, mxx = INT_MIN, mny = INT_MAX, mxy = INT_MIN;
#pragma unroll
    for (int k = 0; k < M::kPx; ++k) {
        const int ix = sat16(sx[k] >> M::kShift), iy = sat16(sy[k] >> M::kShift);
        mnx = min(mnx, ix);
        mxx = max(mxx, ix);
        mny = min(mny, iy);
        mxy = max(mxy, iy);
    }
    mnx = __reduce_min_sync(0xffffffffu, mnx);
    mxx = __reduce_max_sync(0xffffffffu, mxx);
    mny = __reduce_min_sync(0xffffffffu, mny);
    mxy = __reduce_max_sync(0xffffffffu, mxy);
    if (store) s_red[warp] = make_int4(mnx, mxx, mny, mxy);
}
__device__ __forceinline__ int4 block_box_load(const int4* s_red, int lane) {
    int4 r = make_int4(INT_MAX, INT_MIN, INT_MAX, INT_MIN);
    if (lane < kSamplers / 32) r = s_red[lane];
    r.x = __reduce_min_sync(0xffffffffu, r.x);
    r.y = __reduce_max_sync(0xffffffffu, r.y);
    r.z = __reduce_min_sync(0xffffffffu, r.z);
    r.w = __reduce_max_sync(0xffffffffu, r.w);
    return r;
}

template <class M>
__device__ __forceinline__ int box_rsel(int nrows) {
    return nrows <= M::kRowsMin ? 0 : (nrows - M::kRowsMin + kRowsStep - 1) / kRowsStep;
}
struct TileRect {
    int bx0, wbytes;
    int ry0, nrows;
    int rsel, box_rows;
};
template <class M>
__device__ __forceinline__ TileRect tile_rect(int mnx, int mxx, int mny, int mxy) {
    TileRect r;
    r.bx0 = (3 * (mnx - M::kLo)) & ~15;
    r.wbytes = ((3 * (mxx + M::kHi + 1) + 15) & ~15) - r.bx0;
    r.ry0 = mny - M::kLo;
    r.nrows = mxy + M::kHi + 1 - r.ry0;
    r.rsel = box_rsel<M>(r.nrows);
    r.box_rows = M::kRowsMin + r.rsel * kRowsStep;
    return r;
}

template <class M>
__device__ __forceinline__ void pitch_costs(int sx0, int sy0, const TileRect& rc, int pitch0, int lane, int* s_cost) {
    const int row = (sy0 >> M::kShift) - M::kLo - rc.ry0, col = 3 * ((sx0 >> M::kShift) - M::kLo) - rc.bx0;
    int cost = 0;
#pragma unroll
    for (int e = 0; e < kPitchCands; ++e) {
        const int w = (row * (pitch0 + kPitchStep * e) + col) >> 2;
        const unsigned same = __match_any_sync(0xffffffffu, w);
        const bool leader = (__ffs(same) - 1) == lane;
        const unsigned lm = __ballot_sync(0xffffffffu, leader);
        int deg = 0;
        if (leader) deg = __popc(__match_any_sync(lm, w & 31));
        deg = __reduce_max_sync(0xffffffffu, deg);
        if (lane == e) cost = deg;
    }
    constexpr int kStepsPerWarp = M::kTileH * kTileW / kSamplers;
    constexpr int kLoads = M::kInterp == VR180_INTER_NEAREST ? 2 : M::kInterp == VR180_INTER_LINEAR ? 6
                         : M::kInterp == VR180_INTER_CUBIC ? 16 : 56;
    if (lane < kPitchCands) atomicAdd(&s_cost[lane], cost * (kStepsPerWarp * kLoads));
}
template <class Fits>
__device__ __forceinline__ int pick_pitch(const int* s_cost, int pitch0, int box_rows, Fits fits) {
    int best = 0, best_cost = INT_MAX;
#pragma unroll
    for (int e = 0; e < kPitchCands; ++e) {
        const int pe = pitch0 + kPitchStep * e;
        const int c = s_cost[e] + box_rows * pe / 64;
        if (pe <= kPitchMax && fits(pe) && c < best_cost) { best_cost = c; best = e; }
    }
    return pitch0 + kPitchStep * best;
}

template <class M>
__device__ __forceinline__ void gather_pixel(const RemapArgs& a, int f, int i, int j, int v_begin, int v_end, int qx, int qy,
                                             const short* tab) {
    uint8_t* drow = a.dst + (long long)f * a.dst_frame_stride + (long long)j * a.dst_pitch;
    for (int v = v_begin; v < v_end; ++v) {
        const ViewArgs& vw = a.view[v];
        Src s{vw.src + (long long)f * vw.frame_stride, vw.rows, vw.cols, vw.pitch};
        int px[3];
        if (M::kInterp == VR180_INTER_NEAREST)
            fetch_tap<3>(s, sat16(qx), sat16(qy), a.border_mode, a.bv, px);
        else if (M::kInterp == VR180_INTER_LINEAR)
            sample_linear<3>(s, qx, qy, a.border_mode, a.bv, px);
        else if (M::kInterp == VR180_INTER_CUBIC)
            sample_tab<3, 4>(s, qx, qy, tab, a.border_mode, a.bv, px);
        else
            sample_tab<3, 8>(s, qx, qy, tab, a.border_mode, a.bv, px);
        uint8_t* o = drow + (long long)(vw.dst_x_offset + i) * 3;
        o[0] = (uint8_t)px[0];
        o[1] = (uint8_t)px[1];
        o[2] = (uint8_t)px[2];
    }
}

template <class M, int FR>
__device__ __forceinline__ void sample_item(uint32_t sbuf, uint32_t frame_bytes, const typename M::Pixel& p, uint32_t pitch,
                                            uint32_t (&out)[FR]) {
    if constexpr (M::kInterp == VR180_INTER_LANCZOS4) {
        M::template sample_frames<FR>(sbuf, frame_bytes, p, pitch, out);
    } else {
#pragma unroll
        for (int f = 0; f < FR; ++f) out[f] = M::sample(sbuf + f * frame_bytes, p, pitch);
    }
}

inline int zero_border(const RemapArgs& a) {
    return (a.border_mode == VR180_BORDER_CONSTANT && !(a.bv[0] | a.bv[1] | a.bv[2])) ? 1 : 0;
}
template <auto Kernel>
int max_dyn_smem_once(int bytes, int& dev) {
    static std::atomic<int> done[64];
    dev = 0;
    VR180_CUDA(cudaGetDevice(&dev));
    if (dev < 64 && !done[dev].load(std::memory_order_acquire)) {
        VR180_CUDA(cudaFuncSetAttribute(Kernel, cudaFuncAttributeMaxDynamicSharedMemorySize, bytes));
        done[dev].store(1, std::memory_order_release);
    }
    return VR180_OK;
}

}

const tiled::TmaMaps* tma_maps_for(const RemapArgs& a0, int interp, int rows_min, int tile_h, int fr);
int tiled_debug_flags();
int launch_remap_stream(const RemapArgs& a, int interp, const short* weight_tab, cudaStream_t st);
}
```

Before: 734,400.

## Make tile width per-mode and use 64x16 tiles for bilinear sampling

Replaces the global 32-pixel tile width with a per-interpolation kTileW and switches the bilinear mode to 64x16 tiles (kRowsMin lowered to 18). Warp-to-pixel mapping, trig tables, output staging, TMA store boxes and packed LUT sizing are generalised to handle the new shape. A wider, shorter tile is meant to make source-row staging and output TMA stores cover longer contiguous runs and shrink the vertical footprint each CTA fetches. In exchange, the source bounding box per tile changes shape, which can raise or lower staged bytes depending on the warp geometry, and layout code becomes more complex.

```diff
diff --git a/vr180-convert_b200/csrc/chain_fast.cuh b/vr180-convert_b200/csrc/chain_fast.cuh
--- a/vr180-convert_b200/csrc/chain_fast.cuh
+++ b/vr180-convert_b200/csrc/chain_fast.cuh
@@ -117,21 +117,20 @@
     return az <= 1.0 ? th : CUDART_NAN;
 }
 
-constexpr int kStdTableDoubles = 7 * 32;
 __device__ __forceinline__ void std_tables(const double* R, bool lat_is_y, bool is_row, double sv, double cv, double* x_side,
-                                           double* y_side, int idx) {
+                                           double* y_side, int stride, int idx) {
     const bool is_x = lat_is_y == is_row;
     if (is_x) {
         const int o = lat_is_y ? 1 : 0;
         x_side[idx] = cv;
-        x_side[32 + idx] = R[o] * sv;
-        x_side[64 + idx] = R[3 + o] * sv;
-        x_side[96 + idx] = R[6 + o] * sv;
+        x_side[stride + idx] = R[o] * sv;
+        x_side[2 * stride + idx] = R[3 + o] * sv;
+        x_side[3 * stride + idx] = R[6 + o] * sv;
     } else {
         const int o = lat_is_y ? 0 : 1;
         y_side[idx] = fma(R[o], sv, R[2] * cv);
-        y_side[32 + idx] = fma(R[3 + o], sv, R[5] * cv);
-        y_side[64 + idx] = fma(R[6 + o], sv, R[8] * cv);
+        y_side[stride + idx] = fma(R[3 + o], sv, R[5] * cv);
+        y_side[2 * stride + idx] = fma(R[6 + o], sv, R[8] * cv);
     }
 }
 
diff --git a/vr180-convert_b200/csrc/stream.cu b/vr180-convert_b200/csrc/stream.cu
--- a/vr180-convert_b200/csrc/stream.cu
+++ b/vr180-convert_b200/csrc/stream.cu
@@ -11,7 +11,7 @@
 struct SLay {
     static constexpr int kSlotBytes = kStreamSlotBytes<M>;
     static_assert(kSlots == 3, "kStreamSlotBytes (tiled.cuh) is a third of the staging area");
-    static constexpr int kOutTileBytes = M::kTileH * kTileW * 3;
+    static constexpr int kOutTileBytes = M::kTileH * M::kTileW * 3;
     static constexpr int kOB = kOutBufs;
     static constexpr int kOutItemBytes = 2 * kOutTileBytes;
     static constexpr int kOffOut = kSlots * kSlotBytes;
@@ -65,10 +65,10 @@
     const int tid = threadIdx.x, lane = tid & 31, sw = tid >> 5;
     const ViewArgs& mv = a.view[grp];
     const int ty = tile / sp.tiles_x, tx = tile - ty * sp.tiles_x;
-    const int x0 = tx * kTileW, y0 = ty * M::kTileH;
+    const int x0 = tx * M::kTileW, y0 = ty * M::kTileH;
 #pragma unroll
     for (int k = 0; k < kPx; ++k) {
-        const int i = x0 + lane, j = y0 + kPx * sw + k;
+        const int i = x0 + px_col<M>(sw, lane), j = y0 + px_row<M>(sw, k);
         if (i >= a.W || j >= a.H) continue;
         int2 q;
         if (packed) {
@@ -140,8 +140,8 @@
             const int ty = tile / sp.tiles_x, tx = tile - ty * sp.tiles_x;
             const CUtensorMap* const map0 = &tm.src[grp][(g.pitch - kPitchMin) / kPitchStep][g.rsel];
             const int n_rects = a.n_frames * nv, per_item = 2 * g.eye_pitch <= kSlotBytes ? 2 : 1;
-            const int x_l = (a.view[grp].dst_x_offset + tx * kTileW) * 3;
-            const int x_r = nv == 2 ? (a.view[grp + 1].dst_x_offset + tx * kTileW) * 3 : x_l;
+            const int x_l = (a.view[grp].dst_x_offset + tx * M::kTileW) * 3;
+            const int x_r = nv == 2 ? (a.view[grp + 1].dst_x_offset + tx * M::kTileW) * 3 : x_l;
             for (int r = 0; r < n_rects; r += per_item) {
                 if (n_load - n_store == kSlots) store_next();
                 const uint32_t bar = s_full + l_slot * 8;
@@ -165,7 +165,7 @@
     const int sw = warp;
     const int sub = lane & 3;
     const uint32_t out_sel = sub == 0 ? 0x4210u : (sub == 1 ? 0x5421u : 0x6542u);
-    uint32_t outp = s_out + (kPx * sw) * (kTileW * 3) + (3 * (lane >> 2) + sub) * 4;
+    uint32_t outp = s_out + px_row<M>(sw, 0) * (M::kTileW * 3) + 3 * px_col<M>(sw, 0) + (3 * (lane >> 2) + sub) * 4;
     uint32_t flags = (sub != 3 ? 1u : 0u) | (lane == 0 ? 2u : 0u);
     asm volatile("" : "+r"(outp), "+r"(flags));
 
@@ -241,7 +241,7 @@
                     if (v == 0 && n >= kOB) mbar_wait(s_oempty + o * 8, (uint32_t)(n / kOB + 1) & 1u);
                     if (flags & 1u) {
 #pragma unroll
-                        for (int k = 0; k < kPx; ++k) sts32(ob + v * kOutTileBytes + k * (kTileW * 3), word[k]);
+                        for (int k = 0; k < kPx; ++k) sts32(ob + v * kOutTileBytes + k * (M::kTileW * 3), word[k]);
                     }
                 }
                 fence_proxy_async();
@@ -277,7 +277,7 @@
 static int launch_stream_mode(const RemapArgs& a, const short* tab, cudaStream_t st) {
     const int n_groups = a.share_map ? 1 : a.n_views;
     if (a.n_frames > 0x7fff) return VR180_ERR_UNSUPPORTED;
-    const TmaMaps* tm = tma_maps_for(a, M::kInterp, M::kRowsMin, M::kTileH, 1);
+    const TmaMaps* tm = tma_maps_for(a, M::kInterp, M::kRowsMin, M::kTileW, M::kTileH, 1);
     if (!tm) return VR180_ERR_UNSUPPORTED;
     int dev = 0;
     const int rc = max_dyn_smem_once<k_warp_stream<M>>(SLay<M>::kSmemBytes, dev);
@@ -290,7 +290,7 @@
     }
     StreamParams sp;
     memset(&sp, 0, sizeof(sp));
-    sp.tiles_x = (a.W + kTileW - 1) / kTileW;
+    sp.tiles_x = (a.W + M::kTileW - 1) / M::kTileW;
     const long long tiles = (long long)sp.tiles_x * ((a.H + M::kTileH - 1) / M::kTileH);
     if (tiles * n_groups > 0x7fffffffLL) return VR180_ERR_UNSUPPORTED;
     sp.n_tiles = (int)tiles;
diff --git a/vr180-convert_b200/csrc/tiled.cu b/vr180-convert_b200/csrc/tiled.cu
--- a/vr180-convert_b200/csrc/tiled.cu
+++ b/vr180-convert_b200/csrc/tiled.cu
@@ -16,7 +16,7 @@
                                            const double (&nx)[M::kPx], const double (&ny)[M::kPx], const short* tab) {
     static_assert(FR == 1 || !DYN, "a per-frame radius gives every frame its own rectangle");
     static_assert(M::kOutTiles / FR >= 2, "at least two out buffers of one item each");
-    constexpr int kOutTileBytes = M::kTileH * kTileW * 3;
+    constexpr int kOutTileBytes = M::kTileH * M::kTileW * 3;
     constexpr int kOutItemBytes = FR * kOutTileBytes;
     constexpr int OB = M::kOutTiles / FR < kOutBufs ? M::kOutTiles / FR : kOutBufs;
     const int tid = threadIdx.x, lane = tid & 31, warp = tid >> 5;
@@ -98,10 +98,10 @@
     const int sub = lane & 3;
     const uint32_t out_sel = sub == 0 ? 0x4210u : (sub == 1 ? 0x5421u : 0x6542u);
     const bool writer = sub != 3;
-    constexpr int kOutStep = M::kRowPatch ? kTileW * 3 : 24;
+    constexpr int kOutStep = M::kRowPatch ? M::kTileW * 3 : 24;
     const int sw = band * (4 / M::kPx) + cg;
-    uint32_t outp = s_out + (M::kRowPatch ? (M::kPx * sw) * (kTileW * 3) + (3 * (lane >> 2) + sub) * 4
-                                          : (4 * band + (lane >> 3)) * (kTileW * 3) + M::kPx * cg * 24 +
+    uint32_t outp = s_out + (M::kRowPatch ? px_row<M>(sw, 0) * (M::kTileW * 3) + 3 * px_col<M>(sw, 0) + (3 * (lane >> 2) + sub) * 4
+                                          : (4 * band + (lane >> 3)) * (M::kTileW * 3) + M::kPx * cg * 24 +
                                                 (3 * ((lane & 7) >> 2) + sub) * 4);
     uint32_t flags = (writer ? 1u : 0u) | (lane == 0 ? 2u : 0u);
     asm volatile("" : "+r"(outp), "+r"(flags));
@@ -174,6 +174,8 @@
     }
 }
 
+static_assert(4 * (Lay<LinearP>::kSmemBytes + 1024) <= 228 * 1024 && 4 * (Lay<Nearest>::kSmemBytes + 1024) <= 228 * 1024,
+              "4 bilinear / nearest CTAs per SM");
 template <class M, bool DYN, int FR>
 __global__ void __launch_bounds__(kThreads, 4)
 k_warp_tiled(const __grid_constant__ RemapArgs a, const __grid_constant__ vr180_chain_t chain0,
@@ -196,7 +198,7 @@
     int* const s_cost = reinterpret_cast<int*>(smem + Lay<M>::kOffCost);
     if (tid < kPitchCands) s_cost[tid] = 0;
     const int tx = blockIdx.x, ty = blockIdx.y, tile = ty * tp.tiles_x + tx;
-    const int x0 = tx * kTileW, y0 = ty * M::kTileH;
+    const int x0 = tx * M::kTileW, y0 = ty * M::kTileH;
     const bool two_groups = !a.share_map && a.n_views == 2;
     const int g = two_groups ? (int)(blockIdx.z & 1u) : 0;
     const int chunk = two_groups ? (int)(blockIdx.z >> 1) : (int)blockIdx.z;
@@ -205,10 +207,10 @@
     const int f0 = chunk * a.frames_per_cta, f1 = min(a.n_frames, f0 + a.frames_per_cta);
     const bool sampler = warp < kSamplers / 32;
     const int sw = warp & (kSamplers / 32 - 1), band = sw / kWarpsPerBand, cg = sw % kWarpsPerBand;
-    const int lx = M::kRowPatch ? lane : 8 * kPx * cg + (lane & 7), ly = M::kRowPatch ? kPx * sw : 4 * band + (lane >> 3);
+    const int lx = M::kRowPatch ? px_col<M>(sw, lane) : 8 * kPx * cg + (lane & 7), ly = M::kRowPatch ? px_row<M>(sw, 0) : 4 * band + (lane >> 3);
     auto pcol = [&](int k) { return M::kRowPatch ? lx : lx + 8 * k; };
     auto prow = [&](int k) { return M::kRowPatch ? ly + k : ly; };
-    const bool full_tile = (x0 + kTileW <= a.W) && (y0 + M::kTileH <= a.H);
+    const bool full_tile = (x0 + M::kTileW <= a.W) && (y0 + M::kTileH <= a.H);
 
     TileHdr hdr = {0, 0, 0, 0, 0};
     if (mv.map_kind != VR180_MAPSRC_ANALYTIC && mv.packed) hdr = decode_header(packed_header_raw(mv.packed, tile));
@@ -227,26 +229,28 @@
         const StdChain& sc = tp.std[mv.chain_idx ? 1 : 0];
         const bool fastc = sc.valid && sc.fast && !(tp.debug & 256);
         if (sc.valid || tp.sep_prefix) {
-            if (tid < 64) {
-                const bool is_row = tid >= 32;
-                const int idx = tid & 31;
+            if (tid < M::kTileW + M::kTileH) {
+                const bool is_row = tid >= M::kTileW;
+                const int idx = tid & (M::kTileW - 1);
+                const int stride = is_row ? M::kTileH : M::kTileW;
                 const double* nm = ch.ops[0].p;
                 const double c = (double)((is_row ? y0 : x0) + idx);
                 const double n = mul_rn(__ddiv_rn(add_rn(c, -(is_row ? nm[1] : nm[0])), nm[2]), 2.0);
                 double sv, cv;
                 sincos(mul_rn(n, kHalfPi), &sv, &cv);
                 if (fastc) {
-                    std_tables(sc.R, sc.lat_is_y != 0, is_row, sv, cv, s_trig, s_trig + 128, idx);
+                    const int n_x = sc.lat_is_y ? M::kTileH : M::kTileW;
+                    std_tables(sc.R, sc.lat_is_y != 0, is_row, sv, cv, s_trig, s_trig + 4 * n_x, stride, idx);
                 } else {
-                    s_trig[(is_row ? 64 : 0) + idx] = sv;
-                    s_trig[(is_row ? 96 : 32) + idx] = cv;
+                    s_trig[(is_row ? 2 * M::kTileW : 0) + idx] = sv;
+                    s_trig[(is_row ? 2 * M::kTileW + M::kTileH : M::kTileW) + idx] = cv;
                 }
             }
             __syncthreads();
             const bool lat_is_y = ch.ops[1].iparam != 0;
             auto seed = [&](int k, ChainState& s) {
-                const double s_row = s_trig[64 + prow(k)], c_row = s_trig[96 + prow(k)];
-                const double s_col = s_trig[pcol(k)], c_col = s_trig[32 + pcol(k)];
+                const double s_row = s_trig[2 * M::kTileW + prow(k)], c_row = s_trig[2 * M::kTileW + M::kTileH + prow(k)];
+                const double s_col = s_trig[pcol(k)], c_col = s_trig[M::kTileW + pcol(k)];
                 s.mode = MODE_VEC3;
                 s.x = s.y = s.r = s.ux = s.uy = 0.0;
                 if (lat_is_y) {
@@ -264,17 +268,20 @@
                 auto std_eval = [&](const StdChain& c) {
                     const bool x_fixed = M::kRowPatch ? !c.lat_is_y : (c.lat_is_y != 0);
                     const int fi = M::kRowPatch ? lx : ly;
-                    const double* const ft = s_trig + (x_fixed ? 0 : 128) + fi;
-                    const double f0 = ft[0], f1 = ft[32], f2 = ft[64], f3 = x_fixed ? ft[96] : 0.0;
+                    constexpr int fs = M::kRowPatch ? M::kTileW : M::kTileH, vs = M::kRowPatch ? M::kTileH : M::kTileW;
+                    const int y_off = 4 * (x_fixed ? fs : vs);
+                    const double* const ft = s_trig + (x_fixed ? 0 : y_off) + fi;
+                    const double f0 = ft[0], f1 = ft[fs], f2 = ft[2 * fs], f3 = x_fixed ? ft[3 * fs] : 0.0;
 #pragma unroll(kChainUnroll)
                     for (int k = 0; k < kPx; ++k) {
                         const int vi = M::kRowPatch ? prow(k) : pcol(k);
                         double vx, vy, vz;
                         if (x_fixed) {
-                            vx = fma(f0, s_trig[128 + vi], f1); vy = fma(f0, s_trig[160 + vi], f2); vz = fma(f0, s_trig[192 + vi], f3);
+                            const double* const vt = s_trig + y_off + vi;
+                            vx = fma(f0, vt[0], f1); vy = fma(f0, vt[vs], f2); vz = fma(f0, vt[2 * vs], f3);
                         } else {
                             const double sc_ = s_trig[vi];
-                            vx = fma(sc_, f0, s_trig[32 + vi]); vy = fma(sc_, f1, s_trig[64 + vi]); vz = fma(sc_, f2, s_trig[96 + vi]);
+                            vx = fma(sc_, f0, s_trig[vs + vi]); vy = fma(sc_, f1, s_trig[2 * vs + vi]); vz = fma(sc_, f2, s_trig[3 * vs + vi]);
                         }
                         double ox, oy;
                         int qx = 0, qy = 0;
@@ -532,13 +539,13 @@
     __shared__ int s_cost[kPitchCands];
     const int tid = threadIdx.x, lane = tid & 31, sw = tid >> 5;
     const int tx = blockIdx.x % tiles_x, ty = blockIdx.x / tiles_x;
-    const int x0 = tx * kTileW, y0 = ty * M::kTileH;
-    const bool full_tile = (x0 + kTileW <= W) && (y0 + M::kTileH <= H);
+    const int x0 = tx * M::kTileW, y0 = ty * M::kTileH;
+    const bool full_tile = (x0 + M::kTileW <= W) && (y0 + M::kTileH <= H);
     if (tid < kPitchCands) s_cost[tid] = 0;
     int sx[kPx], sy[kPx];
 #pragma unroll
     for (int k = 0; k < kPx; ++k) {
-        const int i = x0 + lane, j = y0 + kPx * sw + k;
+        const int i = x0 + px_col<M>(sw, lane), j = y0 + px_row<M>(sw, k);
         sx[k] = sy[k] = (int)0x80000000;
         if (i < W && j < H) {
             sx[k] = M::quant(__ldg(xmap + (long long)j * map_pitch + i));
@@ -581,27 +588,34 @@
 
 }
 
-static int tile_height_of(int interp) {
-    return interp == VR180_INTER_LINEAR || interp == VR180_INTER_NEAREST ? tiled::LinearP::kTileH
-           : interp == VR180_INTER_CUBIC                                  ? tiled::Cubic::kTileH
-           : interp == VR180_INTER_LANCZOS4                               ? tiled::Lanczos4::kTileH
-                                                                          : 0;
+static long long tile_count_of(int interp, int W, int H, int* tiles_x = nullptr, int* tile_px = nullptr) {
+    auto count = [&](auto mode) {
+        using M = decltype(mode);
+        const int tx = (W + M::kTileW - 1) / M::kTileW;
+        if (tiles_x) *tiles_x = tx;
+        if (tile_px) *tile_px = M::kTileW * M::kTileH;
+        return (long long)tx * ((H + M::kTileH - 1) / M::kTileH);
+    };
+    return interp == VR180_INTER_NEAREST    ? count(tiled::Nearest{})
+           : interp == VR180_INTER_LINEAR   ? count(tiled::LinearP{})
+           : interp == VR180_INTER_CUBIC    ? count(tiled::Cubic{})
+           : interp == VR180_INTER_LANCZOS4 ? count(tiled::Lanczos4{})
+                                            : 0;
 }
 
 size_t packed_lut_bytes(int out_w, int out_h, int interp) {
-    const int th = tile_height_of(interp);
-    if (!th) return 0;
-    const long long n_tiles = (long long)((out_w + tiled::kTileW - 1) / tiled::kTileW) * ((out_h + th - 1) / th);
-    return tiled::packed_entries_offset(n_tiles) + (size_t)n_tiles * tiled::kTileW * th * 4;
+    int tile_px = 0;
+    const long long n_tiles = tile_count_of(interp, out_w, out_h, nullptr, &tile_px);
+    if (!n_tiles) return 0;
+    return tiled::packed_entries_offset(n_tiles) + (size_t)n_tiles * tile_px * 4;
 }
 
 int launch_pack_lut_tiles(const float* xmap, const float* ymap, int64_t map_pitch, int W, int H, int interp, void* packed,
                           cudaStream_t st) {
     using namespace tiled;
-    const int th = tile_height_of(interp);
-    if (!th) return VR180_ERR_UNSUPPORTED;
-    const int tiles_x = (W + kTileW - 1) / kTileW, tiles_y = (H + th - 1) / th;
-    const long long n_tiles = (long long)tiles_x * tiles_y;
+    int tiles_x = 0;
+    const long long n_tiles = tile_count_of(interp, W, H, &tiles_x);
+    if (!n_tiles) return VR180_ERR_UNSUPPORTED;
     if (n_tiles > 0x7fffffffLL) return VR180_ERR_UNSUPPORTED;
     const dim3 grid((unsigned)n_tiles);
     if (interp == VR180_INTER_NEAREST)
@@ -703,7 +717,7 @@
     return fpc;
 }
 
-const tiled::TmaMaps* tma_maps_for(const RemapArgs& a0, int interp, int rows_min, int tile_h, int fr) {
+const tiled::TmaMaps* tma_maps_for(const RemapArgs& a0, int interp, int rows_min, int tile_w, int tile_h, int fr) {
     using namespace tiled;
     struct Key {
         const void* src[2];
@@ -761,7 +775,7 @@
                         return nullptr;
         }
         if (a0.n_views == 1) memcpy(&t.src[1], &t.src[0], sizeof(t.src[0]));
-        if (!encode_u8_3d(&t.dst, a0.dst, a0.dst_pitch, a0.H, a0.n_frames, a0.dst_pitch, a0.dst_frame_stride, kTileW * 3,
+        if (!encode_u8_3d(&t.dst, a0.dst, a0.dst_pitch, a0.H, a0.n_frames, a0.dst_pitch, a0.dst_frame_stride, tile_w * 3,
                           tile_h, fr))
             return nullptr;
         hit->key = key;
@@ -775,7 +789,7 @@
                        cudaStream_t st) {
     using namespace tiled;
     const int n_groups = a0.share_map ? 1 : a0.n_views;
-    const TmaMaps* tmp = tma_maps_for(a0, M::kInterp, M::kRowsMin, M::kTileH, DYN ? 1 : FR);
+    const TmaMaps* tmp = tma_maps_for(a0, M::kInterp, M::kRowsMin, M::kTileW, M::kTileH, DYN ? 1 : FR);
     if (!tmp) return VR180_ERR_UNSUPPORTED;
     const TmaMaps& tm = *tmp;
 
@@ -786,7 +800,7 @@
     RemapArgs a = a0;
     TiledParams tp;
     memset(&tp, 0, sizeof(tp));
-    const int tiles_x = (a.W + kTileW - 1) / kTileW, tiles_y = (a.H + M::kTileH - 1) / M::kTileH;
+    const int tiles_x = (a.W + M::kTileW - 1) / M::kTileW, tiles_y = (a.H + M::kTileH - 1) / M::kTileH;
     tp.tiles_x = tiles_x;
     tp.n_tiles = tiles_x * tiles_y;
     tp.tab = tab;
@@ -864,8 +878,7 @@
             if (rc != VR180_ERR_UNSUPPORTED) return rc;
         }
     }
-    const int tile_h = tile_height_of(interp);
-    const long long tiles = (long long)((a0.W + tiled::kTileW - 1) / tiled::kTileW) * ((a0.H + tile_h - 1) / tile_h) * n_groups;
+    const long long tiles = tile_count_of(interp, a0.W, a0.H) * n_groups;
     const int fpc = frames_per_cta(tiles, a0.n_frames, a0.share_map ? a0.n_views : 1);
     if (interp == VR180_INTER_NEAREST) return launch_tiled<tiled::Nearest>(a0, c0, c1, nullptr, dyn, fpc, st);
     if (interp == VR180_INTER_LINEAR) return launch_tiled<tiled::LinearP>(a0, c0, c1, nullptr, dyn, fpc, st);
diff --git a/vr180-convert_b200/csrc/tiled.cuh b/vr180-convert_b200/csrc/tiled.cuh
--- a/vr180-convert_b200/csrc/tiled.cuh
+++ b/vr180-convert_b200/csrc/tiled.cuh
@@ -14,7 +14,6 @@
 namespace vr180 {
 namespace tiled {
 
-constexpr int kTileW = 32;
 constexpr int kSamplers = 256;
 constexpr int kThreads = kSamplers + 32;
 constexpr int kMaxStages = 8;
@@ -27,10 +26,11 @@
 template <class M>
 struct Lay {
     static constexpr int kStageArea = M::kStageArea;
-    static constexpr int kOutArea = M::kOutTiles * M::kTileH * kTileW * 3;
+    static constexpr int kOutArea = M::kOutTiles * M::kTileH * M::kTileW * 3;
     static constexpr int kOffOut = kStageArea;
     static constexpr int kOffTrig = kOffOut + kOutArea;
-    static constexpr int kOffRed = kOffTrig + 7 * 32 * 8;
+    static constexpr int kTrigDoubles = 4 * (M::kTileW > M::kTileH ? M::kTileW : M::kTileH) + 3 * (M::kTileW > M::kTileH ? M::kTileH : M::kTileW);
+    static constexpr int kOffRed = kOffTrig + kTrigDoubles * 8;
     static constexpr int kOffBar = kOffRed + 8 * 4 * 4;
     static constexpr int kOffOrg = kOffBar + (2 * kMaxStages + 2 * kOutBufs) * 8;
     static constexpr int kOffExt = kOffOrg + kMaxStages * 8;
@@ -168,7 +168,7 @@
 }
 
 struct LinearP {
-    static constexpr int kPx = 4, kTileH = 32, kLo = 0, kHi = 1, kRowsMin = 32, kInterp = VR180_INTER_LINEAR;
+    static constexpr int kPx = 4, kTileW = 64, kTileH = 16, kLo = 0, kHi = 1, kRowsMin = 18, kInterp = VR180_INTER_LINEAR;
     static constexpr int kShift = kInterBits;
     __device__ static __forceinline__ int quant(float m) { return quantise(m); }
     static constexpr int kStageArea = kStageAreaDefault, kWeightSmem = 0, kOutTiles = 4;
@@ -215,7 +215,7 @@
 };
 
 struct Nearest {
-    static constexpr int kPx = 4, kTileH = 32, kLo = 0, kHi = 0, kRowsMin = 32, kInterp = VR180_INTER_NEAREST;
+    static constexpr int kPx = 4, kTileW = 32, kTileH = 32, kLo = 0, kHi = 0, kRowsMin = 32, kInterp = VR180_INTER_NEAREST;
     static constexpr int kShift = 0;
     __device__ static __forceinline__ int quant(float m) { return cv_round(m); }
     static constexpr int kStageArea = kStageAreaDefault, kWeightSmem = 0, kOutTiles = 4;
@@ -237,7 +237,7 @@
 };
 
 struct Cubic {
-    static constexpr int kPx = 2, kTileH = 16, kLo = 1, kHi = 2, kRowsMin = 16, kInterp = VR180_INTER_CUBIC;
+    static constexpr int kPx = 2, kTileW = 32, kTileH = 16, kLo = 1, kHi = 2, kRowsMin = 16, kInterp = VR180_INTER_CUBIC;
     static constexpr int kShift = kInterBits;
     __device__ static __forceinline__ int quant(float m) { return quantise(m); }
     static constexpr int kStageArea = kStageAreaDefault, kWeightSmem = 0, kOutTiles = 8;
@@ -280,7 +280,7 @@
 };
 
 struct Lanczos4 {
-    static constexpr int kPx = 1, kTileH = 8, kLo = 3, kHi = 4, kRowsMin = 16, kInterp = VR180_INTER_LANCZOS4;
+    static constexpr int kPx = 1, kTileW = 32, kTileH = 8, kLo = 3, kHi = 4, kRowsMin = 16, kInterp = VR180_INTER_LANCZOS4;
     static constexpr bool kRowPatch = true;
     static constexpr int kShift = kInterBits;
     __device__ static __forceinline__ int quant(float m) { return quantise(m); }
@@ -368,6 +368,16 @@
 }
 
 template <class M>
+__host__ __device__ constexpr int px_col(int sw, int lane) { return 32 * (sw % (M::kTileW / 32)) + lane; }
+template <class M>
+__host__ __device__ constexpr int px_row(int sw, int k) { return M::kPx * (sw / (M::kTileW / 32)) + k; }
+template <class M>
+constexpr bool tile_shape_ok() {
+    return (M::kTileW == 32 || M::kTileW == 64) && M::kTileH <= M::kTileW && M::kTileH * M::kTileW == kSamplers * M::kPx;
+}
+static_assert(tile_shape_ok<LinearP>() && tile_shape_ok<Nearest>() && tile_shape_ok<Cubic>() && tile_shape_ok<Lanczos4>(),
+              "8 sampling warps x kPx steps cover the tile; the TMA store box is <= 256 bytes wide");
+template <class M>
 __device__ __forceinline__ void block_box_store(const int (&sx)[M::kPx], const int (&sy)[M::kPx], int4* s_red, int warp,
                                                 bool store) {
     int mnx = INT_MAX, mxx = INT_MIN, mny = INT_MAX, mxy = INT_MIN;
@@ -431,7 +441,7 @@
         deg = __reduce_max_sync(0xffffffffu, deg);
         if (lane == e) cost = deg;
     }
-    constexpr int kStepsPerWarp = M::kTileH * kTileW / kSamplers;
+    constexpr int kStepsPerWarp = M::kTileH * M::kTileW / kSamplers;
     constexpr int kLoads = M::kInterp == VR180_INTER_NEAREST ? 2 : M::kInterp == VR180_INTER_LINEAR ? 6
                          : M::kInterp == VR180_INTER_CUBIC ? 16 : 56;
     if (lane < kPitchCands) atomicAdd(&s_cost[lane], cost * (kStepsPerWarp * kLoads));
@@ -499,7 +509,7 @@
 
 }
 
-const tiled::TmaMaps* tma_maps_for(const RemapArgs& a0, int interp, int rows_min, int tile_h, int fr);
+const tiled::TmaMaps* tma_maps_for(const RemapArgs& a0, int interp, int rows_min, int tile_w, int tile_h, int fr);
 int tiled_debug_flags();
 int launch_remap_stream(const RemapArgs& a, int interp, const short* weight_tab, cudaStream_t st);
 }
```

After: 746,500, median of 6. 1.6% higher.
